# thelondonsmiths/Solex_ser_recon_EN

Hardware: AMD Instinct MI355X
Metric: SER frames/sec end-to-end (decode→clahe) + %HBM roofline, 1/2/4/8 MI355X (higher is better)
Workload: dtype u16

## Files before the change

### solex_ser_recon_en_amd/Solex_recon.py

```python
import contextlib
import functools
import math
import os
import queue
import sys
import threading

import numpy as np

from . import dist, ops, outputs, timing
from .device import DeviceImage, bind_thread, cpu_plan, default_device, to_device_u16
from .ellipse_to_circle import correct_image, ellipse_to_circle
from .fits_io import write_fits
from . import stages
from .solex_util import (as_uint16_image, clearlog, compute_mean_return_fit, correct_transversalium2_batch, extract_disks,
                         image_process_batch, logme, make_header, output_path, plots_enabled, removeVignette, savgol_taps,
                         savgol_window, write_complete, write_products)
from .video_reader import video_reader


WORKERS = 4


def _worker_count(workers, n_tasks):
# ... 498 lines not shown
                except BaseException as e:
                    with lock:
                        state['errors'].append((i, e))
                    break
            stream.synchronize()

    for k in range(n_workers):
        _Service.named('shg-scan-%s-%d' % (device, k)).jobs.put(functools.partial(run, k))
    for _ in range(n_workers):
        done.acquire()
    if state['errors']:
        raise min(state['errors'], key=lambda ie: ie[0])[1]


def _one_call_ok(rdr, options):
    if os.environ.get('SHG_SCAN_CALL', '1') == '0' or timing.enabled:
        return False
    if options.get('_shard_frames') or dist.is_sharded(rdr):
        return False
    if options['de-vignette'] or (options['transversalium'] and options.get('stubborn_transversalium')):
        return False
    return True


def scan_one_call(rdr, options):
    return _OneCall(rdr, options).run().finish()


class _OneCall:

    def __init__(self, rdr, options, pooled=False):
        self.rdr, self.options = rdr, options
        self.basefich0 = basefich0 = os.path.splitext(str(rdr.file))[0]
        options['basefich0'] = basefich0
        self.log = log = basefich0 + '_log.txt'
        clearlog(log, options)
        logme(log, options, 'Pixel shift : ' + str(options['shift']))
        options['shift_requested'] = options['shift']
        options['shift'] = list(dict.fromkeys([options['ellipse_fit_shift'], 0] + options['shift']))
        self.hdr = make_header(rdr)
        logme(log, options, 'Width, Height : ' + str(rdr.Width) + ' ' + str(rdr.Height))
        logme(log, options, 'Number of frames : ' + str(rdr.FrameCount))
        self.shifts = shifts = options['shift']
        self.requested = [sh in options['shift_requested'] for sh in shifts]
        self.plots = plots = plots_enabled(options)
        self.call = stages.ScanCall(rdr.device_stack(), shifts, self.requested, options, savgol_taps, want_plot_data=plots,
                                    want_fit_image=plots, own_buffers=pooled)

    def run(self):
        self.call.run()
        return self

    def submit(self, pool):
        self.call.submit(pool)
        return self

    def done(self):
        return self.call.done()

    def finish(self):
        from .ellipse_to_circle import _log_geometry, _warp_geometry
        rdr, options, hdr, log, basefich0 = self.rdr, self.options, self.hdr, self.log, self.basefich0
        shifts, requested, plots = self.shifts, self.requested, self.plots
        r, error = self.call.wait().collect()
        self.call = None
        _release_stack(rdr)
        phase = r['phase']
        if phase >= 1:
            mean_img = DeviceImage(r['mean'])
            y1, y2 = r['y1'], r['y2']
            if options['save_fit']:
                outputs.submit(write_fits, output_path(basefich0 + '_mean.fits', options), mean_img, hdr)
            logme(log, options, 'Vertical limits y1, y2 : ' + str(y1) + ' ' + str(y2))
            logme(log, options, lambda: 'Spectral line polynomial fit: ' + str(r['p']))
            if plots:
                rows = np.arange(y1, y2)
                good = r['mask_good']
                outputs.submit(outputs.plot_spectral_line, output_path(basefich0 + '_spectral_line_data.png', options), mean_img,
                               r['sharp'].astype(np.int64)[y1:y2][good], rows[good], r['fit'][:, 3], int(rdr.ih), (y2 - y1) // 20 + 1)
        disk_list = []
        if phase >= 2:
            hdr['NAXIS1'] = rdr.iw
            if options['save_fit'] or plots or (phase >= 3 and not r['limb_fitted'] and requested[0] and '_nolog' not in options):
                disk_list = [DeviceImage(r['disks'][i], minmax=r['extrema'][i]) for i in range(len(shifts))]
            if options.get('_keep_raw'):
                options['_raw_disks'] = [DeviceImage(r['disks'][i]) for i in range(len(shifts))]
            for i, disk in enumerate(disk_list):
                if options['save_fit'] and requested[i]:
                    outputs.submit(write_fits, output_path(basefich0 + '_shift=' + str(shifts[i]) + '_raw.fits', options), disk, hdr)
            if options['transversalium']:
                logme(log, options, 'Transversalium correction : ' + str(options['trans_strength']))
            else:
                logme(log, options, 'Transversalium disabled')
            logme(log, options, 'Mirror X : ' + str(options['flip_x']))
            logme(log, options, 'Post-rotation : ' + str(options['img_rotate']) + ' degrees')
            logme(log, options, f'Protus adjustment : {options["delta_radius"]}')
            logme(log, options, f'de-vignette : {options["de-vignette"]}')
        if phase >= 3:
            if r['limb_fitted']:
                options['ratio_fixe'] = r['ratio']
                _log_geometry(options, r['phi'], r['ratio'], r['theta_first'], np.array(r['circle'][:2]), r['circle'][2])
                print('sun borders found:' + str(r['borders']))
                options['slant_fix'] = math.degrees(r['phi'])
            elif requested[0] and '_nolog' not in options:
                ih_, n_ = disk_list[0].shape
                theta, inv_mat, _, _, _, origin, det = _warp_geometry(float(r['phi']), float(r['ratio']), int(ih_), int(n_))
                _log_geometry(options, r['phi'], r['ratio'], theta, (inv_mat @ np.array([-1.0, -1.0]).T).T - origin,
                              -1.0 * np.sqrt(np.abs(r['ratio'] / det)), known=False)
        if error is not None:
            raise error
        names = [basefich0 + '_shift=' + str(shifts[i]) for i in range(len(shifts)) if requested[i]]
        if plots and r['limb_fitted']:
            fix_img = r['frames'][0] if requested[0] else r['fit_image']
            outputs.submit(outputs.plot_ellipse_fit, output_path(basefich0 + '_shift=' + str(shifts[0]) + '_ellipse_fit.png', options),
                           disk_list[0], DeviceImage(fix_img), r['raw_X'], r['X_f'], r['outline'], r['borders'])
        if options['save_fit']:
            for j, basefich in enumerate(names):
                outputs.submit(write_fits, output_path(basefich + '_circular.fits', options), DeviceImage(r['frames'][j]), hdr)
        if options['transversalium']:
            for i, basefich in enumerate(names):
                c = r['factors'][i]
                options['_transversalium_cache'] = c
                if plots:
                    outputs.submit(outputs.plot_transversalium, output_path(basefich + '_transversalium_correction.png', options), c)
                if options['save_fit']:
                    outputs.submit(write_fits, output_path(basefich + '_detransversaliumed.fits', options), DeviceImage(r['detrans'][i]), hdr)
        if '_nolog' in options and not options['save_fit'] and options['img_rotate'] // 90 % 4 == 0:
            return [(DeviceImage(r['cc'][i]), DeviceImage(r['protus'][i])) for i in range(len(names))]
        results = [write_products(r['final'][i], r['cl1'][i], r['hc'][i], r['protus'][i], r['cc'][i], options, hdr, names[i])
                   for i in range(len(names))]
        for _ in names:
            write_complete(log, options)
        return results


def _writes_files(options):
    return not (options.get('_shard_frames') and dist.rank() != options.get('_owner', 0))


def solex_read(file, options):
    rdr = file if hasattr(file, 'device_stack') else video_reader(file)
    basefich0 = os.path.splitext(str(rdr.file))[0]
    options['basefich0'] = basefich0
    wopts = options if _writes_files(options) else dict(options, _nolog=True, save_fit=False)
    clearlog(basefich0 + '_log.txt', wopts)
    logme(basefich0 + '_log.txt', wopts, 'Pixel shift : ' + str(options['shift']))
    options['shift_requested'] = options['shift']
    options['shift'] = list(dict.fromkeys([options['ellipse_fit_shift'], 0] + options['shift']))
    if options.get('_shard_frames') and getattr(rdr, '_stack', None) is None:
        rdr.frame_range = dist.frame_block(int(rdr.FrameCount))
    hdr = make_header(rdr)
    ih, iw = rdr.ih, rdr.iw

    with timing.stage('mean_max+line_fit'):
        mean_img, fit, backup_y1, backup_y2 = compute_mean_return_fit(rdr, wopts, hdr, iw, ih, basefich0)
    with timing.stage('extract'):
        disks, extrema = extract_disks(rdr, fit, options['shift'], flip_x=bool(options['flip_x']), want_minmax=True,
                                       owner=options.get('_mosaic_to'))
    hdr['NAXIS1'] = iw

    disk_list = [DeviceImage(disks[i], minmax=None if extrema is None else extrema[i]) for i in range(disks.shape[0])]
    for i, disk in enumerate(disk_list):
        basefich = basefich0 + '_shift=' + str(options['shift'][i])
        flag_requested = options['shift'][i] in options['shift_requested']
        if wopts['save_fit'] and flag_requested:
            outputs.submit(write_fits, output_path(basefich + '_raw.fits', options), disk, hdr)
    return disk_list, (backup_y1, backup_y2), hdr
# ... 176 lines not shown
```

### solex_ser_recon_en_amd/csrc/extract.hip

```cpp
#include <stdlib.h>
#include <algorithm>
#include <type_traits>
#include "shg_common.h"

namespace shg {
thread_local bool t_minmax_slots_zeroed = false;
thread_local void* t_zero_with_fold = nullptr;
thread_local size_t t_zero_with_fold_words = 0;
thread_local void* t_prezeroed = nullptr;
}

namespace {

constexpr int TY = 64;
constexpr int TK = 64;
constexpr int TKP = TK + 2;
constexpr int SC_MAX = 4;

struct ExtractArgs {
    const void* stack;
    int n_frames;
    int64_t height, width, fstride;
    const int32_t* ind_l;
    const double *lw, *rw;
    int n_shifts;
    uint16_t* disks;
    int64_t row_pitch, plane_stride, n_cols, k_offset;
    int flip_x, vec_store;
    uint32_t* mm;
};

template <typename T, bool ROT, int BATCH, int SC> __global__ __launch_bounds__(256) void k_extract(const ExtractArgs kargs) {
    const T* __restrict__ stack = static_cast<const T*>(kargs.stack);
    const int n_frames = kargs.n_frames, n_shifts = kargs.n_shifts, flip_x = kargs.flip_x, vec_store = kargs.vec_store;
    const int64_t height = kargs.height, width = kargs.width, fstride = kargs.fstride, row_pitch = kargs.row_pitch, plane_stride = kargs.plane_stride,
                  n_cols = kargs.n_cols, k_offset = kargs.k_offset;
    const int32_t* __restrict__ ind_l = kargs.ind_l;
    const double* __restrict__ lw = kargs.lw;
    const double* __restrict__ rw = kargs.rw;
    uint16_t* __restrict__ disks = kargs.disks;
    uint32_t* __restrict__ mm = kargs.mm;
    __shared__ uint16_t tile[SC][TY][TKP];
    const int64_t ih = ROT ? width : height;
    const int lane = threadIdx.x & 63;
    const int wave = __builtin_amdgcn_readfirstlane(threadIdx.x >> 6);
    const int64_t c0 = (int64_t)blockIdx.x * TK;
    const int64_t y = (int64_t)blockIdx.y * TY + lane;
    const int s0 = blockIdx.z * SC;
    const int ns = min(SC, n_shifts - s0);
    const bool y_ok = y < ih;
    constexpr int scale = sizeof(T) == 1 ? 256 : 1;

    const int64_t yc = y_ok ? y : ih - 1;
    int il[SC];
    const double wl = lw[yc], wr = rw[yc];
    const double kl = wl * 0x1p+52, kr = wr * 0x1p+52;
    const bool fast = __all(fabs(wl) < 0x1p+900 && fabs(wr) < 0x1p+900) != 0;
#pragma unroll
    for (int s = 0; s < SC; ++s) il[s] = ind_l[(int64_t)(s0 + min(s, ns - 1)) * ih + yc];

    uint32_t off[SC], offr[SC];
    const int64_t step = ROT ? width : 1;
#pragma unroll
    for (int s = 0; s < SC; ++s) {
        off[s] = (uint32_t)((ROT ? (int64_t)il[s] * width + (width - 1 - yc) : yc * width + il[s]) * (int64_t)sizeof(T));
        offr[s] = off[s] + (uint32_t)(step * (int64_t)sizeof(T));
    }

    __shared__ uint32_t wred[4][SC][2];
    uint32_t vlo[SC], vhi[SC];
#pragma unroll
    for (int s = 0; s < SC; ++s) { vlo[s] = 0xffffu; vhi[s] = 0u; }

    for (int cb = wave; cb < TK; cb += 4 * BATCH) {
        T lv[BATCH][SC], rv[BATCH][SC];
        bool ok[BATCH];
#pragma unroll
        for (int i = 0; i < BATCH; ++i) {
            const int cc = cb + 4 * i;
            const int64_t col = c0 + cc;
            const int64_t k = (flip_x ? (n_cols - 1 - col) : col) - k_offset;
            ok[i] = cc < TK && col < n_cols && k >= 0 && k < n_frames;
            const char* f = reinterpret_cast<const char*>(stack + (ok[i] ? k : 0) * fstride);
#pragma unroll
            for (int s = 0; s < SC; ++s) {
                lv[i][s] = *reinterpret_cast<const T*>(f + off[s]);
                rv[i][s] = *reinterpret_cast<const T*>(f + offr[s]);
            }
        }
        auto blend = [&](auto fast_form) {
#pragma unroll
            for (int i = 0; i < BATCH; ++i) {
// ... 356 lines not shown
    constexpr int SEGS = TK / 8;
    const int seg = lane % SEGS;
    const int64_t col = c0 + seg * 8;
    const int64_t ka = (flip_x ? (n_cols - 1 - col) : col) - k_offset;
    const int64_t kb = (flip_x ? (n_cols - 1 - (col + 7)) : (col + 7)) - k_offset;
    const bool whole = a.vec_store && col + 8 <= n_cols && ka >= 0 && ka < n_frames && kb >= 0 && kb < n_frames;
    const int rows_here = (int)min((int64_t)TY, ih - (int64_t)by * TY);
    for (int d = wave; d < ns; d += NW) {
        const int plane = CONSEC ? a.plane_of[g0 + d] : g0 + d;
        uint16_t* dst0 = a.disks + (int64_t)plane * a.plane_stride + ((int64_t)by * TY) * a.row_pitch + col;
        uint32_t lo = 0xffffffffu, hi = 0u;
        if (whole) {
#pragma unroll 4
            for (int r = lane / SEGS; r < rows_here; r += 64 / SEGS) {
                const uint32_t* s32 = &btile[(d * TY + r) * DKW + seg * 4];
                const u32x4_t o = {s32[0], s32[1], s32[2], s32[3]};
                __builtin_nontemporal_store(o, reinterpret_cast<u32x4_t*>(dst0 + r * a.row_pitch));
                lo = pk_min_u16(pk_min_u16(lo, o.x), pk_min_u16(pk_min_u16(o.y, o.z), o.w));
                hi = pk_max_u16(pk_max_u16(hi, o.x), pk_max_u16(pk_max_u16(o.y, o.z), o.w));
            }
        } else {
            for (int r = lane / SEGS; r < rows_here; r += 64 / SEGS) {
                const uint16_t* src = reinterpret_cast<const uint16_t*>(&btile[(d * TY + r) * DKW + seg * 4]);
                uint16_t* dst = dst0 + r * a.row_pitch;
                for (int j = 0; j < 8; ++j) {
                    const int64_t cj = col + j;
                    const int64_t kj = (flip_x ? (n_cols - 1 - cj) : cj) - k_offset;
                    if (cj < n_cols && kj >= 0 && kj < n_frames) {
                        dst[j] = src[j];
                        lo = pk_min_u16(lo, src[j] * 0x10001u);
                        hi = pk_max_u16(hi, src[j] * 0x10001u);
                    }
                }
            }
        }
        if (a.mm) {
            lo = shg::wave_fold_u32(lo, [](uint32_t x, uint32_t y) { return pk_min_u16(x, y); });
            hi = shg::wave_fold_u32(hi, [](uint32_t x, uint32_t y) { return pk_max_u16(x, y); });
            const uint32_t l16 = min(lo & 0xffffu, lo >> 16), h16 = max(hi & 0xffffu, hi >> 16);
            if (lane == 0 && h16 >= l16) {
                const int slot = (int)((bx * 5u + by * 3u) & 63u);
                uint32_t* m = a.mm + ((int64_t)plane * 64 + slot) * 2;
                atomicMax(&m[0], 0xffffu - l16);
                atomicMax(&m[1], h16);
            }
        }
    }
}

template <bool CONSEC>
int launch_band(const BandArgs& ba, int bytes_per_px, int64_t ih, hipStream_t st) {
    const int S = ba.S;
    int G;
    if (CONSEC) {
        const int ng7 = (S + 6) / 7;
        G = std::max(4, (S + ng7 - 1) / ng7);
    } else {
        G = S <= 2 ? 2 : 4;
    }
    const int ng = (S + G - 1) / G;
    const dim3 grid(8u * (unsigned)ng, ((unsigned)ba.nx + 7u) / 8u, (unsigned)((ih + TY - 1) / TY));
    int status = SHG_E_UNSUPPORTED;
#define SHG_BAND(T, GV)                                                                                                                   \
    if (G == GV && bytes_per_px == (int)sizeof(T)) {                                                                                      \
        constexpr size_t lds = (size_t)GV * TY * (TK / 2 + 1) * 4;                                                                        \
        static const bool ok_ = lds <= 64 * 1024 || hipFuncSetAttribute(reinterpret_cast<const void*>(k_extract_band<T, GV, CONSEC>),    \
                                                                        hipFuncAttributeMaxDynamicSharedMemorySize, (int)lds) == hipSuccess; \
        if (!ok_) (void)hipGetLastError();                                                                                                \
        status = shg::launch_timed("extract", k_extract_band<T, GV, CONSEC>, grid, dim3(64 * BAND_NW), lds, st, nullptr, "k_extract_band", ba); \
    }
    if constexpr (CONSEC) {
        SHG_BAND(uint16_t, 4) SHG_BAND(uint16_t, 5) SHG_BAND(uint16_t, 6) SHG_BAND(uint16_t, 7)
        SHG_BAND(uint8_t, 4) SHG_BAND(uint8_t, 5) SHG_BAND(uint8_t, 6) SHG_BAND(uint8_t, 7)
    } else {
        SHG_BAND(uint16_t, 2) SHG_BAND(uint16_t, 4) SHG_BAND(uint8_t, 2) SHG_BAND(uint8_t, 4)
    }
#undef SHG_BAND
    return status;
}

struct FoldMinmaxArgs {
    const uint32_t* slots;
    uint32_t* out;
    int n_planes;
    uint32_t* zero;
    size_t zero_words;
};

__global__ __launch_bounds__(64) void k_fold_minmax(const FoldMinmaxArgs kargs) {
    const uint32_t* __restrict__ slots = kargs.slots;
    uint32_t* __restrict__ out = kargs.out;
    if ((int)blockIdx.x >= kargs.n_planes) {
        uint32_t* __restrict__ z = kargs.zero;
        const size_t stride = (size_t)(gridDim.x - kargs.n_planes) * 64;
        for (size_t i = (size_t)(blockIdx.x - kargs.n_planes) * 64 + threadIdx.x; i < kargs.zero_words; i += stride) z[i] = 0;
        return;
    }
    uint32_t a = slots[((int64_t)blockIdx.x * 64 + threadIdx.x) * 2], b = slots[((int64_t)blockIdx.x * 64 + threadIdx.x) * 2 + 1];
    a = shg::wave_fold_u32(a, [](uint32_t x, uint32_t y) { return x > y ? x : y; });
    b = shg::wave_fold_u32(b, [](uint32_t x, uint32_t y) { return x > y ? x : y; });
    if (threadIdx.x == 0) { out[blockIdx.x * 2] = 0xffffu - a; out[blockIdx.x * 2 + 1] = b; }
}

int launch_fold(uint32_t* minmax_slots, int n_shifts, hipStream_t st) {
    FoldMinmaxArgs fa{minmax_slots, minmax_slots + (int64_t)n_shifts * 64 * 2, n_shifts, nullptr, 0};
    unsigned extra = 0;
    if (shg::t_zero_with_fold && shg::t_zero_with_fold_words > 0) {
        fa.zero = static_cast<uint32_t*>(shg::t_zero_with_fold);
        fa.zero_words = shg::t_zero_with_fold_words;
        extra = (unsigned)std::min<size_t>((fa.zero_words + 1023) / 1024, 64);
    }
    const int e = shg::launch(k_fold_minmax, dim3((unsigned)n_shifts + extra), dim3(64), 0, st, fa, "k_fold_minmax");
    if (e == 0 && extra) shg::t_prezeroed = shg::t_zero_with_fold;
    shg::t_zero_with_fold = nullptr;
    shg::t_zero_with_fold_words = 0;
    return e;
}

}

extern "C" int shg_extract_columns(const void* stack, int64_t n_frames, int64_t height, int64_t width,
                                   int bytes_per_px, int64_t frame_stride_px, const int32_t* ind_l, const double* lw, const double* rw,
                                   int n_shifts, uint16_t* disks, int64_t row_pitch, int64_t plane_stride,
                                   int64_t n_cols, int64_t k_offset, int flip_x, shg_stream_t stream) {
    return shg_extract_columns_minmax(stack, n_frames, height, width, bytes_per_px, frame_stride_px, ind_l, lw, rw, n_shifts, disks,
                                      row_pitch, plane_stride, n_cols, k_offset, flip_x, nullptr, stream);
}

extern "C" int shg_extract_columns_minmax(const void* stack, int64_t n_frames, int64_t height, int64_t width,
                                          int bytes_per_px, int64_t frame_stride_px, const int32_t* ind_l, const double* lw, const double* rw,
                                          int n_shifts, uint16_t* disks, int64_t row_pitch, int64_t plane_stride,
                                          int64_t n_cols, int64_t k_offset, int flip_x, uint32_t* minmax_slots, shg_stream_t stream) {
    const bool slots_zeroed = shg::t_minmax_slots_zeroed;
    shg::t_minmax_slots_zeroed = false;
    SHG_REQUIRE(stack && ind_l && lw && rw && disks, SHG_E_ARG, "shg_extract_columns: null pointer");
    SHG_REQUIRE(n_frames > 0 && height > 0 && width > 0 && n_shifts > 0, SHG_E_ARG, "shg_extract_columns: empty input");
    SHG_REQUIRE(bytes_per_px == 1 || bytes_per_px == 2, SHG_E_ARG, "shg_extract_columns: bytes_per_px must be 1 or 2");
    SHG_REQUIRE(n_frames < (1ll << 31), SHG_E_UNSUPPORTED, "shg_extract_columns: too many frames");
    SHG_REQUIRE(n_cols >= n_frames && k_offset >= 0 && k_offset + n_frames <= n_cols, SHG_E_ARG,
                "shg_extract_columns: frames [%lld, %lld) do not fit %lld columns", (long long)k_offset,
                (long long)(k_offset + n_frames), (long long)n_cols);
    SHG_REQUIRE(row_pitch >= n_cols, SHG_E_ARG, "shg_extract_columns: row_pitch < n_cols");
    SHG_REQUIRE((height < width ? height : width) >= 2, SHG_E_ARG, "shg_extract_columns: spectral axis needs >= 2 pixels");
    SHG_REQUIRE(frame_stride_px == 0 || frame_stride_px >= height * width, SHG_E_ARG, "shg_extract_columns: frame stride smaller than a frame");
    SHG_REQUIRE(height * width * bytes_per_px < (1ll << 32), SHG_E_UNSUPPORTED, "shg_extract_columns: a frame of %lld x %lld samples is larger than 4 GiB",
                (long long)height, (long long)width);
    const int64_t fstride = frame_stride_px > 0 ? frame_stride_px : height * width;
    const bool rot = width > height;
    const int64_t ih = rot ? width : height;
    const int vec_store = ((reinterpret_cast<uintptr_t>(disks) & 15) == 0) && (row_pitch % 8 == 0) && (plane_stride % 8 == 0);
    static const int sc_env = [] { const char* e = getenv("SHG_EXT_SC"); return e ? atoi(e) : 0; }();
    const int sc = n_shifts <= 2 ? 2 : (sc_env == 2 ? 2 : SC_MAX);
    dim3 grid((unsigned)((n_cols + TK - 1) / TK), (unsigned)((ih + TY - 1) / TY), (unsigned)((n_shifts + sc - 1) / sc));
    hipStream_t st = shg::as_stream(stream);
    const int n = (int)n_frames;
    const ExtractArgs xa{stack, n, height, width, fstride, ind_l, lw, rw, n_shifts, disks, row_pitch, plane_stride, n_cols, k_offset, flip_x, vec_store, minmax_slots};
    int launch_status = 0;
#define EXT_LAUNCH_BS(T, ROT, B, SCV) launch_status = shg::launch_timed("extract", k_extract<T, ROT, B, SCV>, grid, dim3(256), 0, st, nullptr, "k_extract", xa)
#define EXT_LAUNCH_B(T, ROT, B) do { if (sc == 2) EXT_LAUNCH_BS(T, ROT, B, 2); else EXT_LAUNCH_BS(T, ROT, B, 4); } while (0)
#define EXT_LAUNCH(T, ROT)                                                 \
    switch (batch) {                                                       \
        case 1: EXT_LAUNCH_B(T, ROT, 1); break;                            \
        case 2: EXT_LAUNCH_B(T, ROT, 2); break;                            \
        case 8: EXT_LAUNCH_B(T, ROT, 8); break;                            \
        case 16: EXT_LAUNCH_B(T, ROT, 16); break;                          \
        default: EXT_LAUNCH_B(T, ROT, 4); break;                           \
    }
    static const int batch_env = [] { const char* e = getenv("SHG_EXT_BATCH"); return e ? atoi(e) : 0; }();
    const int batch2 = 4;
    const int batch = batch_env > 0 ? batch_env : (n_shifts > SC_MAX ? 8 : (n_shifts <= 2 ? batch2 : 4));
    if (minmax_slots && !slots_zeroed) {
        if (hipError_t e = hipMemsetAsync(minmax_slots, 0, (size_t)n_shifts * 64 * 2 * sizeof(uint32_t), st)) {
            shg::set_error("shg_extract_columns: memset: %s", hipGetErrorString(e));
            return (int)e;
        }
    }
    const bool general_only = [] { const char* e = getenv("SHG_EXT_GENERAL"); return e && atoi(e) != 0; }();
    if (rot && !general_only) {
        BandArgs ba{stack, n, height, width, fstride, ind_l, nullptr, lw, rw, n_shifts, disks, row_pitch, plane_stride, n_cols, k_offset, flip_x, vec_store,
                    minmax_slots, (int)((n_cols + TK - 1) / TK), {}};
        launch_status = launch_band<false>(ba, bytes_per_px, ih, st);
        if (launch_status) return launch_status;
        if (minmax_slots) return launch_fold(minmax_slots, n_shifts, st);
        return 0;
    }
    if (bytes_per_px == 2) {
        if (rot) EXT_LAUNCH(uint16_t, true) else EXT_LAUNCH(uint16_t, false)
    } else {
        if (rot) EXT_LAUNCH(uint8_t, true) else EXT_LAUNCH(uint8_t, false)
    }
#undef EXT_LAUNCH_B
#undef EXT_LAUNCH_BS
#undef EXT_LAUNCH
    if (launch_status) return launch_status;
    if (minmax_slots) return launch_fold(minmax_slots, n_shifts, st);
    return 0;
}

extern "C" int shg_extract_dense_fits(const int32_t* host_shifts, int n_shifts) {
    if (!host_shifts || n_shifts < 3 || n_shifts > DS_MAX) return 0;
    int lo = host_shifts[0], hi = host_shifts[0];
    for (int i = 1; i < n_shifts; ++i) { lo = host_shifts[i] < lo ? host_shifts[i] : lo; hi = host_shifts[i] > hi ? host_shifts[i] : hi; }
    if ((int64_t)hi - lo != n_shifts - 1) return 0;
    bool seen[DS_MAX] = {};
    for (int i = 0; i < n_shifts; ++i) {
        if (seen[host_shifts[i] - lo]) return 0;
        seen[host_shifts[i] - lo] = true;
    }
    return 1;
}

extern "C" int shg_extract_columns_dense(const void* stack, int64_t n_frames, int64_t height, int64_t width, int bytes_per_px,
                                         int64_t frame_stride_px, const int32_t* ind_l, const int32_t* base_col, const double* lw,
                                         const double* rw, const int32_t* host_shifts, int n_shifts, uint16_t* disks, int64_t row_pitch,
                                         int64_t plane_stride, int64_t n_cols, int64_t k_offset, int flip_x, uint32_t* minmax_slots,
                                         shg_stream_t stream) {
    const bool slots_zeroed = shg::t_minmax_slots_zeroed;
    shg::t_minmax_slots_zeroed = false;
    SHG_REQUIRE(stack && ind_l && base_col && lw && rw && host_shifts && disks, SHG_E_ARG, "shg_extract_columns_dense: null pointer");
    SHG_REQUIRE(n_frames > 0 && height > 0 && width > 0, SHG_E_ARG, "shg_extract_columns_dense: empty input");
    SHG_REQUIRE(shg_extract_dense_fits(host_shifts, n_shifts), SHG_E_UNSUPPORTED, "shg_extract_columns_dense: the shifts are not 3..%d consecutive integers", DS_MAX);
    SHG_REQUIRE(bytes_per_px == 1 || bytes_per_px == 2, SHG_E_ARG, "shg_extract_columns_dense: bytes_per_px must be 1 or 2");
    SHG_REQUIRE(n_frames < (1ll << 31), SHG_E_UNSUPPORTED, "shg_extract_columns_dense: too many frames");
    SHG_REQUIRE(n_cols >= n_frames && k_offset >= 0 && k_offset + n_frames <= n_cols, SHG_E_ARG, "shg_extract_columns_dense: frames do not fit the columns");
    SHG_REQUIRE(row_pitch >= n_cols, SHG_E_ARG, "shg_extract_columns_dense: row_pitch < n_cols");
    SHG_REQUIRE((height < width ? height : width) > n_shifts, SHG_E_UNSUPPORTED, "shg_extract_columns_dense: the spectral axis must be wider than the shift range");
    SHG_REQUIRE(frame_stride_px == 0 || frame_stride_px >= height * width, SHG_E_ARG, "shg_extract_columns_dense: frame stride smaller than a frame");
    const int64_t fstride = frame_stride_px > 0 ? frame_stride_px : height * width;
    const bool rot = width > height;
    const int64_t ih = rot ? width : height;
    const int vec_store = ((reinterpret_cast<uintptr_t>(disks) & 15) == 0) && (row_pitch % 8 == 0) && (plane_stride % 8 == 0);
    int lo = host_shifts[0];
    for (int i = 1; i < n_shifts; ++i) lo = host_shifts[i] < lo ? host_shifts[i] : lo;
    PlaneOfOffset po = {};
    for (int i = 0; i < n_shifts; ++i) po.v[host_shifts[i] - lo] = i;
    hipStream_t st = shg::as_stream(stream);
    if (minmax_slots && !slots_zeroed) {
        if (hipError_t e = hipMemsetAsync(minmax_slots, 0, (size_t)n_shifts * 64 * 2 * sizeof(uint32_t), st)) {
            shg::set_error("shg_extract_columns_dense: memset: %s", hipGetErrorString(e));
            return (int)e;
        }
    }
    const int n = (int)n_frames;
    if (rot) {
        BandArgs ba{stack, n, height, width, fstride, ind_l, base_col, lw, rw, n_shifts, disks, row_pitch, plane_stride, n_cols, k_offset, flip_x, vec_store,
                    minmax_slots, (int)((n_cols + TK - 1) / TK), {}};
        for (int i = 0; i < n_shifts; ++i) ba.plane_of[host_shifts[i] - lo] = (uint8_t)i;
        const int launch_status = launch_band<true>(ba, bytes_per_px, ih, st);
        if (launch_status) return launch_status;
        if (minmax_slots) return launch_fold(minmax_slots, n_shifts, st);
        return 0;
    }
    static const int shape = [] { const char* e = getenv("SHG_EXT_DENSE_SHAPE"); return e ? atoi(e) : 0; }();
#define SHG_DENSE(T, ROT, B, NW, DKV)                                                                                                               \
    do {                                                                                                                                            \
        static const bool ok_ = hipFuncSetAttribute(reinterpret_cast<const void*>(k_extract_dense<T, ROT, B, NW, DKV>),                            \
                                                    hipFuncAttributeMaxDynamicSharedMemorySize, 160 * 1024) == hipSuccess;                         \
        if (!ok_) (void)hipGetLastError();                                                                                                          \
        const size_t lds = (size_t)n_shifts * TY * (DKV + 2) * sizeof(uint16_t);                                                                    \
        dim3 grid((unsigned)((n_cols + DKV - 1) / DKV), (unsigned)((ih + TY - 1) / TY));                                                            \
        launch_status = shg::launch_timed("extract", k_extract_dense<T, ROT, B, NW, DKV>, grid, dim3(64 * NW), lds, st, nullptr, "k_extract_dense",      \
                                          static_cast<const T*>(stack), n, height, width, fstride, ind_l, base_col, lw, rw,                       \
                                          n_shifts, po, disks, row_pitch, plane_stride, n_cols, k_offset, flip_x, vec_store, minmax_slots);       \
    } while (0)
#define SHG_DENSE_S(T, ROT)                                                                  \
    do {                                                                                     \
        switch (shape) {                                                                     \
            case 1: SHG_DENSE(T, ROT, 4, 8, 32); break;                                      \
            case 2: SHG_DENSE(T, ROT, 2, 16, 32); break;                                     \
            case 3: SHG_DENSE(T, ROT, 4, 4, 16); break;                                      \
            case 4: SHG_DENSE(T, ROT, 2, 8, 16); break;                                      \
            case 5: SHG_DENSE(T, ROT, 2, 4, 8); break;                                       \
            case 6: SHG_DENSE(T, ROT, 4, 4, 32); break;                                      \
            default: SHG_DENSE(T, ROT, 4, 4, 16); break;                                     \
        }                                                                                    \
    } while (0)
    int launch_status = 0;
    if (bytes_per_px == 2) { if (rot) SHG_DENSE_S(uint16_t, true); else SHG_DENSE_S(uint16_t, false); }
    else { if (rot) SHG_DENSE_S(uint8_t, true); else SHG_DENSE_S(uint8_t, false); }
#undef SHG_DENSE_S
#undef SHG_DENSE
    if (launch_status) return launch_status;
    if (minmax_slots) return launch_fold(minmax_slots, n_shifts, st);
    return 0;
}
```

### solex_ser_recon_en_amd/csrc/limb_fused.hip

```cpp
#include <math.h>
#include <stdlib.h>
#include <algorithm>
#include "shg_common.h"

namespace {

#if defined(__HIP_DEVICE_COMPILE__) && !defined(__gfx950__)
#error "limb_fused.hip: published() relies on how gfx950 performs agent-scope atomics; use an acq_rel agent-scope fetch_add elsewhere"
#endif
__device__ __forceinline__ void published() {
    asm volatile("s_waitcnt vmcnt(0)" ::: "memory");
    __syncthreads();
}
__device__ __forceinline__ bool count_done(uint32_t* done, uint32_t total, int fence) {
    const uint32_t before = fence ? __hip_atomic_fetch_add(done, 1u, __ATOMIC_ACQ_REL, __HIP_MEMORY_SCOPE_AGENT)
                                  : __hip_atomic_fetch_add(done, 1u, __ATOMIC_RELAXED, __HIP_MEMORY_SCOPE_AGENT);
    return before == total - 1;
}
inline int limb_fence() {
    const char* v = getenv("SHG_LIMB_FENCE");
    return v && v[0] == '1';
}


// ... 9 lines not shown
    return (b >> 63) ? ~b : (b | 0x8000000000000000ull);
}
__device__ __forceinline__ double key_f64(uint64_t k) {
    const uint64_t b = (k >> 63) ? (k & 0x7fffffffffffffffull) : ~k;
    return __longlong_as_double((long long)b);
}

struct PrepLayout {
    int bits0, bits1;
    size_t hist0, hist1, coarse0, coarse1, acc, counts, done, zero_words;
    size_t keys5, keysk, total_words;
};

__host__ __device__ inline int bit_length(uint64_t v) {
    int b = 0;
    while (v) { ++b; v >>= 1; }
    return b;
}

PrepLayout prep_layout(int64_t sh, int64_t sw, int k) {
    PrepLayout L;
    const int kk = k > 5 ? k : 5;
    const int total_bits = bit_length((uint64_t)kk * kk * 16ull * 65535ull);
    L.bits1 = total_bits / 2;
    L.bits0 = total_bits - L.bits1;
    size_t off = 0;
    L.hist0 = off; off += (size_t)2 << L.bits0;
    L.hist1 = off; off += (size_t)4 << L.bits1;
    L.coarse0 = off; off += 2 * 256;
    L.coarse1 = off; off += 4 * 256;
    L.acc = off; off += 2 * (4 + 3 * FLOOD_SLOTS + 4 + FLOOD_SLOTS);
    L.counts = off; off += 20;
    L.done = off; off += 4;
    L.zero_words = off;
    off = (off + 63) / 64 * 64;
    const size_t n = (size_t)sh * (size_t)sw;
    L.keysk = off; off += (n + 63) / 64 * 64;
    L.keys5 = off; off += (n + 63) / 64 * 64;
    L.total_words = off;
    return L;
}

__device__ __forceinline__ void flush_hist(const uint32_t* lh, int bits, uint32_t* coarse_lds, uint32_t* __restrict__ fine,
                                           uint32_t* __restrict__ coarse, int tid, int nthreads) {
    for (int e = tid; e < 256; e += nthreads) coarse_lds[e] = 0;
    __syncthreads();
    const int shift = bits - 8;
    for (int e = tid; e < (1 << bits); e += nthreads) {
        const uint32_t c = lh[e];
        if (c) {
            atomicAdd(&fine[e], c);
            atomicAdd(&coarse_lds[e >> shift], c);
        }
    }
    __syncthreads();
    for (int e = tid; e < 256; e += nthreads)
        if (coarse_lds[e]) atomicAdd(&coarse[e], coarse_lds[e]);
}

__device__ __forceinline__ int refl101(int i, int n) {
    if (i < 0) i = -i;
    if (i >= n) i = 2 * n - 2 - i;
    return (i >= 0 && i < n) ? i : (int)shg::reflect101(i, n);
}

constexpr int BT = 16;
constexpr int NT1 = 1024;
struct ZeroWordsArgs {
    uint32_t* dst;
    size_t n_words;
};
__global__ __launch_bounds__(256) void k_zero_words(const ZeroWordsArgs kargs) {
    uint32_t* __restrict__ dst = kargs.dst;
    for (size_t i = (size_t)blockIdx.x * 256 + threadIdx.x; i < kargs.n_words; i += (size_t)gridDim.x * 256) dst[i] = 0;
}

struct LimbBlurArgs {
    const uint16_t* img;
    int h, w;
    int64_t pitch;
    int sh, sw, k, vec4;
    uint32_t *keysk, *keys5;
    unsigned long long* acc;
};
__global__ __launch_bounds__(256) void k_limb_blur(const LimbBlurArgs kargs) {
    const uint16_t* __restrict__ img = kargs.img;
    const int h = kargs.h, w = kargs.w, sh = kargs.sh, sw = kargs.sw, k = kargs.k, vec4 = kargs.vec4;
    const int64_t pitch = kargs.pitch;
    uint32_t* __restrict__ keysk = kargs.keysk;
    uint32_t* __restrict__ keys5 = kargs.keys5;
    unsigned long long* __restrict__ acc = kargs.acc;
    __shared__ uint32_t S[(BT + KMAX) * (BT + KMAX)];
    __shared__ uint32_t H[(BT + KMAX) * BT];
    __shared__ unsigned long long wsum[4];
    __shared__ uint32_t wmin[4];
    const int hl = max(k / 2, 2), hr = max(k - 1 - k / 2, 2);
    const int RH = BT + hl + hr, RW = RH;
    const int x0 = blockIdx.x * BT, y0 = blockIdx.y * BT;
    const int tid = threadIdx.x;
    uint32_t my_min = 0xffffffffu;
    unsigned long long own = 0;
    for (int e = tid; e < RH * RW; e += 256) {
        const int r = e / RW, c = e - r * RW;
        const int sy = refl101(y0 - hl + r, sh), sx = refl101(x0 - hl + c, sw);
        uint32_t s = 0;
        if (vec4 && sx * 4 + 4 <= w && sy * 4 + 4 <= h) {
            uint2 q[4];
#pragma unroll
            for (int j = 0; j < 4; ++j) q[j] = *reinterpret_cast<const uint2*>(img + (int64_t)(sy * 4 + j) * pitch + sx * 4);
#pragma unroll
            for (int j = 0; j < 4; ++j) s += (q[j].x & 0xffffu) + (q[j].x >> 16) + (q[j].y & 0xffffu) + (q[j].y >> 16);
        } else {
            for (int j = 0; j < 4; ++j) {
                const int y = sy * 4 + j;
                if (y >= h) break;
                for (int i = 0; i < 4; ++i) {
                    const int x = sx * 4 + i;
                    if (x < w) s += img[(int64_t)y * pitch + x];
                }
            }
        }
        S[e] = s;
        const int oy = y0 - hl + r, ox = x0 - hl + c;
        if (r >= hl && r < hl + BT && c >= hl && c < hl + BT && oy < sh && ox < sw) own += s;
    }
    own = shg::wave_sum((uint64_t)own);
    if ((tid & 63) == 0) wsum[tid >> 6] = own;
    const int n_arrays = k == 5 ? 1 : 2;
    for (int a = 0; a < n_arrays; ++a) {
        const int kw = a == 0 ? k : 5;
        uint32_t* keys = a == 0 ? keysk : keys5;
        __syncthreads();
        const int c_off = hl - kw / 2, r_lo = hl - kw / 2, r_n = BT + kw - 1;
        for (int e = tid; e < r_n * BT; e += 256) {
            const int r = r_lo + e / BT, x = e % BT;
            uint32_t s = 0;
            for (int j = 0; j < kw; ++j) s += S[r * RW + x + c_off + j];
            H[r * BT + x] = s;
        }
        __syncthreads();
        const int y = tid / BT, x = tid % BT;
        if (y0 + y < sh && x0 + x < sw) {
            uint32_t s = 0;
            for (int j = 0; j < kw; ++j) s += H[(r_lo + y + j) * BT + x];
            keys[(int64_t)(y0 + y) * sw + x0 + x] = s;
            if (a == 0) my_min = s;
        }
    }
    my_min = shg::wave_fold_u32(my_min, [](uint32_t x, uint32_t y) { return x < y ? x : y; });
    if ((tid & 63) == 0) wmin[tid >> 6] = my_min;
    __syncthreads();
    if (tid == 0) {
        const int slot = (blockIdx.y * gridDim.x + blockIdx.x) % FLOOD_SLOTS;
        const unsigned long long t = wsum[0] + wsum[1] + wsum[2] + wsum[3];
        if (t) atomicAdd(&acc[4 + 3 * slot], t);
        const uint32_t m = min(min(wmin[0], wmin[1]), min(wmin[2], wmin[3]));
        if (m != 0xffffffffu) atomicMax(&acc[4 + 3 * FLOOD_SLOTS + 4 + slot], ~f64_key(((double)m * kUnit) * (1.0 / ((double)k * (double)k))));
    }
}

__device__ __forceinline__ void wave_pick(const uint32_t* __restrict__ fine, const uint32_t* __restrict__ coarse, int bits, int64_t rank,
                                          int& digit, int64_t& below) {
    const int lane = threadIdx.x & 63;
    const int per = 1 << (bits - 8);
    int64_t c[4], local = 0;
#pragma unroll
    for (int j = 0; j < 4; ++j) {
        c[j] = __hip_atomic_load(&coarse[lane * 4 + j], __ATOMIC_RELAXED, __HIP_MEMORY_SCOPE_AGENT);
        local += c[j];
    }
    int64_t incl = shg::wave_scan((int64_t)local);
    int64_t excl = incl - local;
    int chunk = -1;
    int64_t base = 0;
    if (excl <= rank && rank < incl) {
#pragma unroll
        for (int j = 0; j < 4; ++j) {
            if (chunk < 0 && rank < excl + c[j]) { chunk = lane * 4 + j; base = excl; }
            excl += c[j];
        }
    }
    const unsigned long long owner = __ballot(chunk >= 0);
    const int src = owner ? __ffsll((long long)owner) - 1 : 0;
    chunk = __shfl(chunk, src);
    base = __shfl(base, src);
    const int64_t f = lane < per ? (int64_t)__hip_atomic_load(&fine[chunk * per + lane], __ATOMIC_RELAXED, __HIP_MEMORY_SCOPE_AGENT) : 0;
    int64_t fi = shg::wave_scan((int64_t)f);
    const int64_t fe = base + fi - f;
    const bool mine = lane < per && fe <= rank && rank < fe + f;
    const unsigned long long who = __ballot(mine);
    const int src2 = who ? __ffsll((long long)who) - 1 : 0;
    digit = chunk * per + src2;
    below = __shfl(fe, src2);
}

struct Ranks4 { int64_t rank[4]; int array[4]; double scale[4]; };

struct LimbSelect0Args {
    const uint32_t *keysk, *keys5;
    int64_t n;
    int bits0, bits1;
    uint32_t *hist0, *coarse0;
};
__global__ __launch_bounds__(256) void k_limb_select0(const LimbSelect0Args kargs) {
    const uint32_t* __restrict__ keysk = kargs.keysk;
    const uint32_t* __restrict__ keys5 = kargs.keys5;
    const int64_t n = kargs.n;
    const int bits0 = kargs.bits0, bits1 = kargs.bits1;
    uint32_t* __restrict__ hist0 = kargs.hist0;
    uint32_t* __restrict__ coarse0 = kargs.coarse0;
    extern __shared__ uint32_t lds[];
    __shared__ uint32_t lc[256];
    const int a = blockIdx.y;
    const uint32_t* __restrict__ v = a ? keys5 : keysk;
    for (int e = threadIdx.x; e < (1 << bits0); e += 256) lds[e] = 0;
    __syncthreads();
    const int64_t stride = (int64_t)gridDim.x * 256;
    for (int64_t base = (int64_t)blockIdx.x * 256 + threadIdx.x; base < n; base += 4 * stride) {
        uint32_t kk[4];
        bool ok[4];
#pragma unroll
        for (int u = 0; u < 4; ++u) { const int64_t i = base + u * stride; ok[u] = i < n; kk[u] = v[ok[u] ? i : 0]; }
#pragma unroll
        for (int u = 0; u < 4; ++u)
            if (ok[u]) atomicAdd(&lds[kk[u] >> bits1], 1u);
    }
    __syncthreads();
    flush_hist(lds, bits0, lc, hist0 + ((size_t)a << bits0), coarse0 + a * 256, threadIdx.x, 256);
}

struct LimbSelect1Args {
    const uint32_t *keysk, *keys5;
    int64_t n;
    Ranks4 p;
    int bits0, bits1;
    const uint32_t *hist0, *coarse0;
    uint32_t *hist1, *coarse1;
    double gamma;
    uint32_t* done;
    unsigned long long* acc;
    double* out4;
    int fence;
};
__global__ __launch_bounds__(256) void k_limb_select1(const LimbSelect1Args kargs) {
    const uint32_t* __restrict__ keysk = kargs.keysk;
    const uint32_t* __restrict__ keys5 = kargs.keys5;
    const int64_t n = kargs.n;
    const Ranks4& p = kargs.p;
    const int bits0 = kargs.bits0, bits1 = kargs.bits1;
    const uint32_t* __restrict__ hist0 = kargs.hist0;
    const uint32_t* __restrict__ coarse0 = kargs.coarse0;
    uint32_t* __restrict__ hist1 = kargs.hist1;
    uint32_t* __restrict__ coarse1 = kargs.coarse1;
    const double gamma = kargs.gamma;
    uint32_t* __restrict__ done = kargs.done;
    unsigned long long* __restrict__ acc = kargs.acc;
    double* __restrict__ out4 = kargs.out4;
    extern __shared__ uint32_t lds[];
    __shared__ uint32_t lc[256];
    __shared__ int last;
    __shared__ double val[4];
    const int pair = blockIdx.y;
    const uint32_t* __restrict__ v = p.array[pair] ? keys5 : keysk;
    int digit;
    int64_t below;
    wave_pick(hist0 + ((size_t)p.array[pair] << bits0), coarse0 + p.array[pair] * 256, bits0, p.rank[pair], digit, below);
    for (int e = threadIdx.x; e < (1 << bits1); e += 256) lds[e] = 0;
    __syncthreads();
    const uint32_t mask = (1u << bits1) - 1u;
    const int64_t stride = (int64_t)gridDim.x * 256;
    for (int64_t base = (int64_t)blockIdx.x * 256 + threadIdx.x; base < n; base += 4 * stride) {
        uint32_t kk[4];
        bool ok[4];
#pragma unroll
        for (int u = 0; u < 4; ++u) { const int64_t i = base + u * stride; ok[u] = i < n; kk[u] = v[ok[u] ? i : 0]; }
#pragma unroll
        for (int u = 0; u < 4; ++u)
            if (ok[u] && (int)(kk[u] >> bits1) == digit) atomicAdd(&lds[kk[u] & mask], 1u);
    }
    __syncthreads();
    flush_hist(lds, bits1, lc, hist1 + ((size_t)pair << bits1), coarse1 + pair * 256, threadIdx.x, 256);
    published();
    if (threadIdx.x == 0) last = count_done(done, gridDim.x * gridDim.y, kargs.fence);
    __syncthreads();
    if (!last) return;
    {
        const int q = threadIdx.x >> 6;
        int d0, d1;
        int64_t b0, b1;
        wave_pick(hist0 + ((size_t)p.array[q] << bits0), coarse0 + p.array[q] * 256, bits0, p.rank[q], d0, b0);
        wave_pick(hist1 + ((size_t)q << bits1), coarse1 + q * 256, bits1, p.rank[q] - b0, d1, b1);
        const uint64_t key = ((uint64_t)d0 << bits1) | (uint64_t)d1;
        if ((threadIdx.x & 63) == 0) val[q] = ((double)key * kUnit) * p.scale[q];
    }
    __syncthreads();
    __shared__ double vb_s;
    __shared__ int scan_s;
    __shared__ unsigned long long wmax[4];
    if (threadIdx.x == 0) {
        const double a = val[2], b = val[3], diff = b - a;
        const double very_bright = gamma >= 0.5 ? b - diff * (1.0 - gamma) : a + diff * gamma;
        out4[0] = val[0]; out4[1] = val[1]; out4[2] = a; out4[3] = b;
        acc[3] = (unsigned long long)__double_as_longlong(very_bright);
        vb_s = very_bright;
        scan_s = !(a < very_bright);
    }
    __syncthreads();
    const double very_bright = vb_s;
    unsigned long long hi = 0ull;
    if (scan_s) {
        const uint32_t* __restrict__ vk = p.array[2] ? keys5 : keysk;
        for (int64_t i = threadIdx.x; i < n; i += 256) {
// ... 351 lines not shown
    if (threadIdx.x == 0) base = part[0] + part[1] + part[2] + part[3];
    __syncthreads();
    for (int xb = 0; xb < w; xb += 256) {
        const int x = xb + threadIdx.x;
        int root = -1, hi = 0;
        if (x < w) {
            const int i = y * w + x;
            const int l = L[i];
            if (l >= 0) {
                root = g_find(L, l);
                hi = (mask[i] >> 1) & 1;
            }
        }
        const unsigned long long m = __ballot(root >= 0);
        if (lane == 0) wave_cnt[wave] = __popcll(m);
        __syncthreads();
        int off = base;
        for (int i = 0; i < wave; ++i) off += wave_cnt[i];
        if (root >= 0) {
            const int pos = off + __popcll(m & ((1ull << lane) - 1ull));
            comp[1 + pos] = y * w + x;
            comp[1 + n + pos] = root | (hi << 30);
        }
        __syncthreads();
        if (threadIdx.x == 0) base += wave_cnt[0] + wave_cnt[1] + wave_cnt[2] + wave_cnt[3];
        __syncthreads();
    }
    if (y == h - 1 && threadIdx.x == 0) comp[0] = base;
}

size_t canny_tile_lds(int R) {
    const int FW = TW + 4 + 2 * R, FH = TH + 4 + 2 * R, VW = FW, VH = TH + 4, SW = TW + 4, MW = TW + 2, MH = TH + 2;
    return (size_t)(((VH + 7) & ~7) + VH * VW + VH * SW + 3 * MH * MW) * 8 + (size_t)TH * TW * 4 + (size_t)FH * FW;
}

}

extern "C" int shg_limb_fused_fits(int64_t sh, int64_t sw, int k) {
    return sh > 2 && sw > 2 && sh * sw < (1ll << 30) && k >= 1 && k <= KMAX;
}

size_t shg::limb_prepare_zero_words(int64_t h, int64_t w) {
    const int64_t sh = (h + 3) / 4, sw = (w + 3) / 4;
    const int k = (int)((double)sh * 0.01);
    if (!shg_limb_fused_fits(sh, sw, k)) return 0;
    return prep_layout(sh, sw, k).zero_words;
}

extern "C" size_t shg_limb_prepare_workspace_bytes(int64_t sh, int64_t sw, int k) {
    if (!shg_limb_fused_fits(sh, sw, k)) return 0;
    return prep_layout(sh, sw, k).total_words * 4;
}

extern "C" int shg_limb_prepare(const uint16_t* img, int64_t h, int64_t w, int64_t pitch, int k, const int64_t* host_ranks4, double gamma99,
                                double* packed, const uint32_t** keys_out, void* workspace, size_t workspace_bytes, shg_stream_t stream) {
    SHG_REQUIRE(img && host_ranks4 && packed && keys_out && workspace, SHG_E_ARG, "shg_limb_prepare: null pointer");
    SHG_REQUIRE(h > 0 && w > 0 && pitch >= w, SHG_E_ARG, "shg_limb_prepare: bad image size");
    const int64_t sh = (h + 3) / 4, sw = (w + 3) / 4, n = sh * sw;
    SHG_REQUIRE(shg_limb_fused_fits(sh, sw, k), SHG_E_UNSUPPORTED, "shg_limb_prepare: a %d x %d window on %lld x %lld is outside the fused path", k, k,
                (long long)sh, (long long)sw);
    SHG_REQUIRE(gamma99 >= 0.0 && gamma99 <= 1.0, SHG_E_ARG, "shg_limb_prepare: gamma %g outside [0, 1]", gamma99);
    const PrepLayout lay = prep_layout(sh, sw, k);
    SHG_REQUIRE(workspace_bytes >= lay.total_words * 4, SHG_E_WORKSPACE, "shg_limb_prepare: workspace too small");
    SHG_REQUIRE((reinterpret_cast<uintptr_t>(workspace) & 7) == 0, SHG_E_ARG, "shg_limb_prepare: workspace not 8-byte aligned");
    for (int i = 0; i < 4; ++i) SHG_REQUIRE(host_ranks4[i] >= 0 && host_ranks4[i] < n, SHG_E_ARG, "shg_limb_prepare: rank outside the image");
    hipStream_t st = shg::as_stream(stream);
    uint32_t* ws = static_cast<uint32_t*>(workspace);
    uint32_t *hist0 = ws + lay.hist0, *hist1 = ws + lay.hist1, *coarse0 = ws + lay.coarse0, *coarse1 = ws + lay.coarse1;
    uint32_t *counts = ws + lay.counts, *done = ws + lay.done;
    unsigned long long* acc = reinterpret_cast<unsigned long long*>(ws + lay.acc);
    uint32_t *keysk = ws + lay.keysk, *keys5 = k == 5 ? keysk : ws + lay.keys5;
    double* out4 = reinterpret_cast<double*>(acc + 4 + 3 * FLOOD_SLOTS);
    SHG_PROF("limb_prepare", st);
    if (shg::t_prezeroed == workspace) {
        shg::t_prezeroed = nullptr;
    } else if (int e = shg::launch(k_zero_words, dim3((unsigned)std::min<size_t>((lay.zero_words + 255) / 256, 64)), dim3(256), 0, st, ZeroWordsArgs{ws, lay.zero_words}, "k_zero_words")) {
        return e;
    }
    Ranks4 p;
    const double scale_k = 1.0 / ((double)k * (double)k), scale_5 = 1.0 / 25.0;
    for (int i = 0; i < 4; ++i) { p.rank[i] = host_ranks4[i]; p.array[i] = (i < 2 && k != 5) ? 1 : 0; p.scale[i] = (i < 2) ? scale_5 : scale_k; }
    dim3 grid1((unsigned)((sw + BT - 1) / BT), (unsigned)((sh + BT - 1) / BT));
    const int vec4 = (reinterpret_cast<uintptr_t>(img) & 7) == 0 && pitch % 4 == 0;
    if (int e = shg::launch(k_limb_blur, grid1, dim3(256), 0, st, LimbBlurArgs{img, (int)h, (int)w, pitch, (int)sh, (int)sw, k, vec4, keysk, keys5, acc}, "k_limb_blur")) return e;
    static const bool lds_ok = [] {
        return hipFuncSetAttribute(reinterpret_cast<const void*>(k_limb_select0), hipFuncAttributeMaxDynamicSharedMemorySize, 128 * 1024) == hipSuccess &&
               hipFuncSetAttribute(reinterpret_cast<const void*>(k_limb_select1), hipFuncAttributeMaxDynamicSharedMemorySize, 128 * 1024) == hipSuccess;
    }();
    if (!lds_ok) (void)hipGetLastError();
    int64_t blocks = (n + 2047) / 2048;
    if (blocks > 256) blocks = 256;
    if (int e = shg::launch(k_limb_select0, dim3((unsigned)blocks, k == 5 ? 1u : 2u), dim3(256), ((size_t)1 << lay.bits0) * 4, st,
                           LimbSelect0Args{keysk, keys5, n, lay.bits0, lay.bits1, hist0, coarse0}, "k_limb_select0"))
        return e;
    if (int e = shg::launch(k_limb_select1, dim3((unsigned)blocks, 4u), dim3(256), ((size_t)1 << lay.bits1) * 4, st,
                           LimbSelect1Args{keysk, keys5, n, p, lay.bits0, lay.bits1, hist0, coarse0, hist1, coarse1, gamma99, done, acc, out4, limb_fence()}, "k_limb_select1"))
        return e;
    *keys_out = keysk;
    return shg::launch(k_limb_flood_hist, dim3((unsigned)blocks), dim3(256), 0, st, LimbFloodHistArgs{keysk, n, scale_k, acc, out4, counts, done + 1, packed, limb_fence()}, "k_limb_flood_hist");
}

extern "C" size_t shg_limb_edges_workspace_bytes(int64_t sh, int64_t sw) {
    if (sh <= 0 || sw <= 0) return 0;
    const size_t n = (size_t)sh * (size_t)sw, tiles_x = (size_t)((sw + TW - 1) / TW);
    return ((n + 255) / 256 * 256) + n * 4 + (size_t)sh * tiles_x * 4 + 256;
}

extern "C" int shg_limb_edges(const uint32_t* keys, int64_t sh, int64_t sw, int k, double flood_thresh, const double* host_gauss_weights,
                              int radius, double low, double high, int32_t* comp, void* workspace, size_t workspace_bytes, shg_stream_t stream) {
    SHG_REQUIRE(keys && host_gauss_weights && comp && workspace, SHG_E_ARG, "shg_limb_edges: null pointer");
    SHG_REQUIRE(sh > 2 && sw > 2 && sh * sw < (1ll << 30) && k >= 1, SHG_E_ARG, "shg_limb_edges: bad image size");
    SHG_REQUIRE(radius >= 0 && radius <= MAXR, SHG_E_UNSUPPORTED, "shg_limb_edges: Gaussian radius %d > %d", radius, MAXR);
    SHG_REQUIRE(workspace_bytes >= shg_limb_edges_workspace_bytes(sh, sw), SHG_E_WORKSPACE, "shg_limb_edges: workspace too small");
    GaussW g;
    g.radius = radius;
    for (int i = 0; i < 2 * radius + 1; ++i) g.w[i] = host_gauss_weights[i];
    const size_t n = (size_t)sh * (size_t)sw;
    const int tiles_x = (int)((sw + TW - 1) / TW);
    uint8_t* mask = static_cast<uint8_t*>(workspace);
    int* L = reinterpret_cast<int*>(mask + (n + 255) / 256 * 256);
    int* row_counts = L + n;
    hipStream_t st = shg::as_stream(stream);
    SHG_PROF("limb_edges", st);
    dim3 grid((unsigned)tiles_x, (unsigned)((sh + TH - 1) / TH));
    static const bool lds_ok = hipFuncSetAttribute(reinterpret_cast<const void*>(k_limb_canny_tile), hipFuncAttributeMaxDynamicSharedMemorySize, 160 * 1024) == hipSuccess;
    if (!lds_ok) (void)hipGetLastError();
    if (int e = shg::launch(k_limb_canny_tile, grid, dim3(NT1), canny_tile_lds(radius), st,
                           LimbCannyArgs{keys, (int)sh, (int)sw, 1.0 / ((double)k * (double)k), flood_thresh, g, low, high, mask, L, row_counts, tiles_x}, "k_limb_canny_tile"))
        return e;
    {
        const int64_t tops = ((sh + TH - 1) / TH) * sw, sides = 2 * (int64_t)tiles_x * sh;
        if (int e = shg::launch(k_limb_border_merge, dim3((unsigned)((std::max(tops, sides) + 255) / 256), 2u), dim3(256), 0, st, LimbBorderArgs{mask, (int)sh, (int)sw, L}, "k_limb_border_merge"))
            return e;
    }
    return shg::launch(k_limb_emit, dim3((unsigned)sh), dim3(256), 0, st, LimbEmitArgs{mask, L, (int)sh, (int)sw, row_counts, tiles_x, (int)n, comp}, "k_limb_emit");
}
```

### solex_ser_recon_en_amd/csrc/scan.hip

```cpp
#include <math.h>
#include <string.h>
#include <atomic>
#include <vector>
#include "shg_common.h"

namespace {

constexpr size_t kAlign = 256;
inline size_t up(size_t b) { return (b + kAlign - 1) / kAlign * kAlign; }
inline int64_t round64(int64_t v) { return (v + 63) / 64 * 64; }
inline int64_t floor_div(int64_t a, int64_t b) { int64_t q = a / b; return (a % b != 0 && ((a < 0) != (b < 0))) ? q - 1 : q; }

const double kRadToDeg = 180.0 / 3.141592653589793238462643383279502884;
const double kDegToRad = 3.141592653589793238462643383279502884 / 180.0;

std::atomic<shg_savgol_taps_fn> g_taps_fn{nullptr};

#define SCAN_TRY(expr)                  \
    do {                                \
        if (int e_ = (expr)) return e_; \
    } while (0)

struct Regions {
    size_t mean_ws, extract_ws, limb_ws, mean_pin, extract_pin, limb_pin, process_pin;
// ... 90 lines not shown
        SHG_REQUIRE(fabs(c[0]) < 9e15 && fabs(c[1]) < 9e15 && fabs(c[2]) < 9e15, SHG_E_VALUE, "cannot convert float NaN / infinity to integer (disk circle)");
        const int64_t r = (int64_t)c[2] + rq->delta_radius;
        if (r > 0) { pl->disc[0] = (int64_t)c[0]; pl->disc[1] = (int64_t)c[1]; pl->disc[2] = r; }
    }
    memcpy(rs->disc3, pl->disc, sizeof(rs->disc3));
    return 0;
}

}

extern "C" int shg_host_set_savgol_taps(shg_savgol_taps_fn fn) {
    g_taps_fn.store(fn);
    return 0;
}

extern "C" size_t shg_scan_workspace_bytes(const shg_scan_request* rq) {
    if (!rq || rq->height <= 0 || rq->width <= 0 || rq->n_frames <= 0 || rq->n_shifts <= 0 || !rq->host_requested) return 0;
    const Regions r = regions(rq);
    return r.mean_ws + r.extract_ws + r.limb_ws + kAlign;
}

extern "C" size_t shg_scan_host_bytes(const shg_scan_request* rq) {
    if (!rq || rq->height <= 0 || rq->width <= 0 || rq->n_frames <= 0 || rq->n_shifts <= 0 || !rq->host_requested) return 0;
    const Regions r = regions(rq);
    return r.mean_pin + r.extract_pin + r.limb_pin + r.process_pin + kAlign;
}

extern "C" int shg_scan_prelaunch(const shg_scan_request* rq, shg_stream_t after, int* launched) {
    SHG_REQUIRE(rq && launched, SHG_E_ARG, "shg_scan_prelaunch: null pointer");
    *launched = 0;
    if (rq->struct_bytes != sizeof(shg_scan_request) || rq->start_phase != 0 || !rq->stack || !rq->workspace || rq->n_frames <= 0 ||
        rq->height <= 0 || rq->width <= 0 || rq->n_shifts <= 0 || (rq->bytes_per_px != 1 && rq->bytes_per_px != 2))
        return 0;
    const Regions rg = regions(rq);
    const size_t acc = shg_accumulate_workspace_bytes(rq->n_frames, rq->height, rq->width, rq->bytes_per_px);
    if (rq->workspace_bytes < rg.mean_ws || acc == 0 || acc > rg.mean_ws) return 0;
    return shg_pass_a_prelaunch(rq->stack, rq->n_frames, rq->height, rq->width, rq->bytes_per_px, rq->frame_stride_px, rq->workspace, acc, after,
                                launched);
}

extern "C" int shg_scan_file(const shg_scan_request* rq, shg_scan_result* rs, shg_stream_t stream) {
    SHG_HOST_TIME("scan_file");
    SHG_REQUIRE(rq && rs, SHG_E_ARG, "shg_scan_file: null pointer");
    SHG_REQUIRE(rq->struct_bytes == sizeof(shg_scan_request), SHG_E_ARG, "shg_scan_file: the caller's shg_scan_request has %u bytes, the library's %zu",
                rq->struct_bytes, sizeof(shg_scan_request));
    SHG_REQUIRE(rq->stack && rq->host_shifts && rq->host_requested && rq->mean_out && rq->max_out && rq->disks && rq->minmax_slots &&
                rq->workspace && rq->host_pinned && rq->host_fit, SHG_E_ARG, "shg_scan_file: null pointer in the request");
    SHG_REQUIRE(rq->n_frames > 0 && rq->height > 0 && rq->width > 0 && rq->n_shifts > 0, SHG_E_ARG, "shg_scan_file: empty input");
    SHG_REQUIRE(rq->disk_pitch >= rq->n_frames && rq->disk_plane_stride > 0, SHG_E_ARG, "shg_scan_file: bad disk layout");
    SHG_REQUIRE(rq->start_phase == 0 || rq->start_phase == 3, SHG_E_ARG, "shg_scan_file: start_phase must be 0 or 3");
    const int64_t ih = slit_rows(rq), n_cols = rq->n_frames;
    const int S = rq->n_shifts;
    const int64_t k = n_requested(rq);
    const bool limb = fits_limb(rq);
    SHG_REQUIRE(!limb || (rq->host_gauss_taps && rq->host_points && rq->host_flags && rq->points_cap > 0), SHG_E_ARG,
                "shg_scan_file: the limb fit needs host_gauss_taps, host_points, host_flags");
    const Regions rg = regions(rq);
    char* ws = static_cast<char*>(rq->workspace);
    char* pin = static_cast<char*>(rq->host_pinned);
    const size_t ws_fixed = rg.mean_ws + rg.extract_ws + rg.limb_ws;
    SHG_REQUIRE(rq->workspace_bytes >= ws_fixed, SHG_E_WORKSPACE, "shg_scan_file: workspace %zu < %zu bytes", rq->workspace_bytes, ws_fixed);
    SHG_REQUIRE(rq->host_pinned_bytes >= rg.mean_pin + rg.extract_pin + rg.limb_pin + rg.process_pin, SHG_E_WORKSPACE,
                "shg_scan_file: pinned staging area %zu < %zu bytes", rq->host_pinned_bytes, rg.mean_pin + rg.extract_pin + rg.limb_pin + rg.process_pin);
    char* mean_ws = ws;
    char* extract_ws = mean_ws + rg.mean_ws;
    char* limb_ws = extract_ws + rg.extract_ws;
    char* process_ws = limb_ws + rg.limb_ws;
    char* mean_pin = pin;
    char* extract_pin = mean_pin + rg.mean_pin;
    char* limb_pin = extract_pin + rg.extract_pin;
    char* process_pin = limb_pin + rg.limb_pin;

    if (rq->start_phase == 0) {
        memset(rs, 0, sizeof(*rs));
        rs->fit_image_off = rs->frames_off = rs->detrans_off = rs->products_off = rs->results_off = -1;
        int64_t y12[2];
        SCAN_TRY(shg_stage_mean_fit(rq->stack, rq->n_frames, rq->height, rq->width, rq->bytes_per_px, rq->frame_stride_px, nullptr, nullptr,
                                    rq->n_frames, rq->mean_out, rq->max_out, y12, rs->p4, rq->host_fit, rq->host_trace_sharp, rq->host_mask_good,
                                    mean_ws, rg.mean_ws, mean_pin, rg.mean_pin, stream));
        rs->y1 = y12[0];
        rs->y2 = y12[1];
        rs->phase_done = 1;
        if (limb) {
            shg::t_zero_with_fold = limb_ws;
            shg::t_zero_with_fold_words = shg::limb_prepare_zero_words(ih, n_cols);
        }
        const int extract_status = shg_stage_extract(rq->stack, rq->n_frames, rq->height, rq->width, rq->bytes_per_px, rq->frame_stride_px, rq->host_fit,
                                                     rq->host_shifts, S, rq->disks, rq->disk_pitch, rq->disk_plane_stride, n_cols, 0, rq->flip_x,
                                                     rq->minmax_slots, extract_ws, rg.extract_ws, extract_pin, rg.extract_pin, stream);
        shg::t_zero_with_fold = nullptr;
        shg::t_zero_with_fold_words = 0;
        if (extract_status) { shg::t_prezeroed = nullptr; return extract_status; }
        rs->phase_done = 2;
        bool later_disks = false;
        for (int i = 1; i < S; ++i) later_disks = later_disks || rq->host_requested[i];
        double mat3[9], inv[4], origin[2], det;
        if (limb) {
            int64_t dims[2];
            const int limb_status = shg_stage_limb_fit(rq->disks, ih, n_cols, rq->disk_pitch, rq->host_gauss_taps, rq->host_points, rq->host_flags, rq->points_cap,
                                                       rs->counts3, rs->geom16, dims, rq->host_outline200, limb_ws, rg.limb_ws, limb_pin, rg.limb_pin, stream);
            shg::t_prezeroed = nullptr;
            if (limb_status) return limb_status;
            const double* g = rs->geom16;
            rs->limb_fitted = 1;
            rs->phi = g[3];
            rs->ratio = g[4];
            memcpy(rs->circle3, g + 5, 3 * sizeof(double));
            memcpy(rs->borders4, g + 8, 4 * sizeof(double));
            memcpy(rs->h_first, g + 12, 3 * sizeof(double));
            rs->theta_first = g[15];
            rs->out_h = dims[0];
            rs->out_w = dims[1];
            memcpy(rs->h_rest, rs->h_first, sizeof(rs->h_rest));
            rs->theta_rest = rs->theta_first;
            if (later_disks) {
                const double phi_again = (rs->phi * kRadToDeg) * kDegToRad;
                int64_t oh, ow;
                SCAN_TRY(shg_host_warp_geometry(phi_again, rs->ratio, ih, n_cols, mat3, inv, origin, &det, &rs->theta_rest, &oh, &ow));
                SHG_REQUIRE(oh == rs->out_h && ow == rs->out_w, SHG_E_VALUE, "process_frames: the frames must share one shape and row pitch");
                memcpy(rs->h_rest, mat3, 3 * sizeof(double));
            }
        } else {
            rs->ratio = isnan(rq->ratio_fixe) ? 1.0 : rq->ratio_fixe;
            rs->phi = isnan(rq->slant_fix_deg) ? 0.0 : rq->slant_fix_deg * kDegToRad;
            SCAN_TRY(shg_host_warp_geometry(rs->phi, rs->ratio, ih, n_cols, mat3, inv, origin, &det, &rs->theta_first, &rs->out_h, &rs->out_w));
            memcpy(rs->h_first, mat3, 3 * sizeof(double));
            memcpy(rs->h_rest, mat3, 3 * sizeof(double));
            rs->theta_rest = rs->theta_first;
            rs->circle3[0] = rs->circle3[1] = rs->circle3[2] = -1;
            shg::t_prezeroed = nullptr;
        }
        rs->phase_done = 3;
    } else {
        SHG_REQUIRE(rs->phase_done == 3, SHG_E_ARG, "shg_scan_file: nothing to resume (phase_done = %d)", rs->phase_done);
    }

    Plan pl;
    SCAN_TRY(make_plan(rq, rs, &pl));
    const int64_t out_h = rs->out_h, out_w = rs->out_w;
    SHG_REQUIRE(out_h > 0 && out_w > 0, SHG_E_VALUE, "correct_image: empty output (%lld x %lld)", (long long)out_h, (long long)out_w);
    const int64_t frame_pitch = round64(out_w);
    const int64_t prod_w = pl.crop_w > 0 ? pl.crop_w : out_w, prod_pitch = round64(prod_w);
    const bool fit_image = rq->want_fit_image && !rq->host_requested[0];
    const bool detrans = rq->transversalium && rq->keep_detrans && k > 0;
    const size_t frame_bytes = up((size_t)out_h * frame_pitch * 2), prod_bytes = up((size_t)out_h * prod_pitch * 2);
    size_t off = 0;
    rs->fit_image_off = fit_image ? (int64_t)off : -1;
    off += fit_image ? frame_bytes : 0;
    rs->frames_off = k > 0 ? (int64_t)off : -1;
    off += (size_t)k * frame_bytes;
    rs->detrans_off = detrans ? (int64_t)off : -1;
    off += detrans ? (size_t)k * frame_bytes : 0;
    rs->products_off = k > 0 ? (int64_t)off : -1;
    off += (size_t)k * 3 * prod_bytes;
    rs->results_off = k > 0 ? 0 : -1;
    rs->needed_results_bytes = (size_t)k * 2 * prod_bytes;
    rs->frame_pitch = frame_pitch;
    rs->n_out = k;
    rs->prod_w = prod_w;
    rs->prod_pitch = prod_pitch;
    rs->needed_arena_bytes = off;
    const size_t process_ws_bytes = k > 0 ? up(shg_stage_process_workspace_bytes(k, out_h, out_w, pl.crop_w, rq->tiles)) : 0;
    rs->needed_workspace_bytes = ws_fixed + process_ws_bytes;
    if (rq->arena_bytes < rs->needed_arena_bytes || (off > 0 && !rq->arena) || rq->results_bytes < rs->needed_results_bytes ||
        (k > 0 && !rq->results) || rq->workspace_bytes < rs->needed_workspace_bytes) {
        shg::set_error("shg_scan_file: the corrected images are %lld x %lld: arena %zu of %zu bytes, results %zu of %zu bytes, workspace %zu of "
                       "%zu bytes -- grow them and call again with start_phase = 3", (long long)out_h, (long long)out_w, rq->arena_bytes,
                       rs->needed_arena_bytes, rq->results_bytes, rs->needed_results_bytes, rq->workspace_bytes, rs->needed_workspace_bytes);
        return SHG_E_WORKSPACE;
    }
    SHG_REQUIRE(((reinterpret_cast<uintptr_t>(rq->arena) | reinterpret_cast<uintptr_t>(rq->results)) & 255) == 0, SHG_E_ARG,
                "shg_scan_file: arenas not 256-byte aligned");
    char* arena = static_cast<char*>(rq->arena);
    char* results = static_cast<char*>(rq->results);
    const uint32_t* extrema = rq->minmax_slots + (size_t)S * 128;
    std::vector<const uint16_t*> w_src;
    std::vector<uint16_t*> w_dst;
    std::vector<const uint32_t*> w_mm;
    std::vector<double> w_h;
    auto add_warp = [&](int i, uint16_t* dst) {
        const double* hr = i == 0 ? rs->h_first : rs->h_rest;
        w_src.push_back(rq->disks + (size_t)i * rq->disk_plane_stride);
        w_dst.push_back(dst);
        w_mm.push_back(extrema + 2 * i);
        w_h.insert(w_h.end(), hr, hr + 3);
    };
    if (fit_image) add_warp(0, reinterpret_cast<uint16_t*>(arena + rs->fit_image_off));
    std::vector<const uint16_t*> frames((size_t)k);
    std::vector<uint16_t*> det((size_t)k), prod[5];
    for (auto& v : prod) v.resize((size_t)k);
    int64_t j = 0;
    for (int i = 0; i < S; ++i) {
        if (!rq->host_requested[i]) continue;
        uint16_t* f = reinterpret_cast<uint16_t*>(arena + rs->frames_off + (size_t)j * frame_bytes);
        add_warp(i, f);
        frames[j] = f;
        if (detrans) det[j] = reinterpret_cast<uint16_t*>(arena + rs->detrans_off + (size_t)j * frame_bytes);
        for (int p = 0; p < 3; ++p) prod[p][j] = reinterpret_cast<uint16_t*>(arena + rs->products_off + ((size_t)j * 3 + p) * prod_bytes);
        for (int p = 0; p < 2; ++p) prod[3 + p][j] = reinterpret_cast<uint16_t*>(results + ((size_t)j * 2 + p) * prod_bytes);
        ++j;
    }
    if (!w_src.empty())
        SCAN_TRY(shg::warp_rows_batch(w_src.data(), (int64_t)w_src.size(), ih, n_cols, rq->disk_pitch, w_h.data(), w_dst.data(), out_h, out_w, frame_pitch,
                                      w_mm.data(), stream));
    if (k > 0) {
        SCAN_TRY(shg_stage_process_frames(frames.data(), k, out_h, out_w, frame_pitch, rq->transversalium, pl.trans_circle, pl.trans_borders,
                                          pl.taps_ptr, pl.window, rq->host_factors, pl.crop_w, pl.sx0, pl.dx0, pl.ncopy, rq->clip_limit, rq->tiles,
                                          pl.disc[0], pl.disc[1], pl.disc[2], detrans ? det.data() : nullptr, frame_pitch, prod[0].data(),
                                          prod[1].data(), prod[2].data(), prod[3].data(), prod[4].data(), prod_pitch, process_ws, process_ws_bytes,
                                          process_pin, rg.process_pin, stream));
    }
    rs->phase_done = 4;
    return 0;
}
```

### solex_ser_recon_en_amd/csrc/shg_common.h

```cpp
#pragma once
#include <hip/hip_runtime.h>
#include <hip/hip_ext.h>
#include <stdint.h>
#include <stdio.h>
#include <type_traits>
#include "../../include/shg_hip.h"

namespace shg {

void set_error(const char* fmt, ...);

inline int check_launch(const char* what) {
    hipError_t e = hipGetLastError();
    if (e != hipSuccess) {
        set_error("%s: %s", what, hipGetErrorString(e));
        return (int)e;
    }
    return 0;
}


template <typename A>
struct same_type { using type = A; };
template <typename A>
inline int launch(void (*k)(A), dim3 grid, dim3 block, size_t lds, hipStream_t st, const typename same_type<A>::type& a, const char* what) {
    hipLaunchKernelGGL(k, grid, block, lds, st, a);
    return check_launch(what);
}

struct TimedEvents { hipEvent_t start = nullptr, stop = nullptr; bool sampled = false; };
int timed_begin(const char* tag, bool want_done, TimedEvents* ev);
void timed_end(const char* tag, hipStream_t st, const TimedEvents& ev, bool launched, hipEvent_t* done);
void event_release(hipEvent_t e);
template <typename... P>
inline int launch_timed(const char* tag, void (*k)(P...), dim3 grid, dim3 block, size_t lds, hipStream_t st, hipEvent_t* done, const char* what,
                        typename same_type<P>::type... a) {
    TimedEvents ev;
    if (int e = timed_begin(tag, done != nullptr, &ev)) return e;
    int r;
    if (ev.start || ev.stop) {
        void* args[] = {static_cast<void*>(&a)...};
        const hipError_t le = hipExtLaunchKernel(reinterpret_cast<const void*>(k), grid, block, args, lds, st, ev.start, ev.stop, 0);
        r = check_launch(what);
        if (r == 0 && le != hipSuccess) { set_error("%s: %s", what, hipGetErrorString(le)); r = (int)le; }
    } else {
        hipLaunchKernelGGL(k, grid, block, lds, st, a...);
        r = check_launch(what);
    }
    timed_end(tag, st, ev, r == 0, done);
    return r;
}

#define SHG_REQUIRE(cond, code, ...)            \
    do {                                        \
        if (!(cond)) {                          \
            shg::set_error(__VA_ARGS__);        \
            return (code);                      \
        }                                       \
    } while (0)

inline hipStream_t as_stream(shg_stream_t s) { return reinterpret_cast<hipStream_t>(s); }

typedef int (*lane_launch_fn)(hipStream_t st, void* arg, hipEvent_t* done);
int on_frame_pass_lane(hipStream_t st, lane_launch_fn launch, void* arg);

extern thread_local bool t_minmax_slots_zeroed;
extern thread_local void* t_zero_with_fold;
extern thread_local size_t t_zero_with_fold_words;
extern thread_local void* t_prezeroed;
size_t limb_prepare_zero_words(int64_t h, int64_t w);
int prelaunch_on_lane(hipStream_t after, lane_launch_fn launch, void* arg, hipEvent_t* done);

struct ProfScope {
    ProfScope(const char* tag, hipStream_t st);
    ~ProfScope();
    int slot;
    hipStream_t stream;
    unsigned generation;
};
#define SHG_PROF(tag, st) shg::ProfScope shg_prof_scope_(tag, st)

struct HostScope {
    explicit HostScope(const char* tag);
    ~HostScope();
    const char* tag;
    double t0;
};
#define SHG_HOST_CAT2(a, b) a##b
#define SHG_HOST_CAT(a, b) SHG_HOST_CAT2(a, b)
#define SHG_HOST_TIME(tag) shg::HostScope SHG_HOST_CAT(shg_host_scope_, __LINE__)(tag)

constexpr int kMaxBatch = 32;
template <int N>
struct PtrBatchN {
    const void* p[N];
    template <typename T>
    __device__ __forceinline__ T* at(int i) const { return static_cast<T*>(const_cast<void*>(p[i])); }
};
using PtrBatch = PtrBatchN<kMaxBatch>;
template <int N, typename T>
inline PtrBatchN<N> make_batch_n(T* const* host_ptrs, int first, int count) {
    PtrBatchN<N> b = {};
    for (int i = 0; i < count && i < N; ++i) b.p[i] = host_ptrs[first + i];
    return b;
}
template <typename T>
inline PtrBatch make_batch(T* const* host_ptrs, int first, int count) { return make_batch_n<kMaxBatch>(host_ptrs, first, count); }

int rowpair_stats_batch(const uint16_t* const* host_imgs, int64_t k, int64_t h, int64_t w, int64_t pitch, int64_t y1, int64_t y2,
                        const int32_t* xa, const int32_t* xb, const double* row_factor, double* out, double* out_mirror, shg_stream_t stream);
int scale_rows_batch(const uint16_t* const* host_imgs, int64_t k, int64_t h, int64_t w, int64_t pitch, const double* c,
                     const double* row_factor, uint16_t* const* host_dsts, int64_t dst_pitch, shg_stream_t stream);
int crop_pad_batch(const uint16_t* const* host_srcs, int64_t k, int64_t h, int64_t w, int64_t pitch, uint16_t* const* host_dsts, int64_t nw,
                   int64_t dst_pitch, int64_t sx0, int64_t dx0, int64_t n, int32_t fill, shg_stream_t stream);
int contrast_products_batch(const uint16_t* const* host_frames, int64_t frame_pitch, const uint16_t* const* host_cl1, int64_t cl1_pitch,
                            int64_t k, int64_t h, int64_t w, const double* host_lo_hi6, uint16_t* const* host_hc, uint16_t* const* host_protus,
                            uint16_t* const* host_cc, int64_t dst_pitch, int64_t disc_x0, int64_t disc_y0, int64_t disc_r, shg_stream_t stream,
                            const double* stats5 = nullptr, double g_bright = 0.0, double g_dark = 0.0, double* mirror5 = nullptr);
int warp_rows_batch(const uint16_t* const* host_srcs, int64_t k, int64_t h, int64_t w, int64_t src_pitch, const double* host_h3,
                    uint16_t* const* host_dsts, int64_t out_h, int64_t out_w, int64_t dst_pitch, const uint32_t* const* host_minmax2,
                    shg_stream_t stream);
struct FrameSource {
    const uint16_t* const* host_raw;
    int64_t raw_pitch;
    const double* factors;
    int64_t sx0, dx0, ncopy;
};
bool contrast_stats_batches(int64_t h, int64_t w, int tiles, double clip_limit);
int contrast_stats_batch(const uint16_t* const* host_frames, int64_t k, int64_t h, int64_t w, int64_t pitch, double clip_limit, int tiles,
                         uint16_t* const* host_cl1, int64_t cl1_pitch, const int64_t* ranks_frame2, const int64_t* ranks_cl13, double* out5,
                         void* workspace, size_t workspace_bytes, shg_stream_t stream, const FrameSource* from = nullptr);

constexpr int kWave = 64;
constexpr int kCUs = 256;

__device__ __forceinline__ int lane_id() { return threadIdx.x & (kWave - 1); }

template <typename Op>
__device__ __forceinline__ uint32_t wave_fold_u32(uint32_t v, Op op) {
    v = op(v, (uint32_t)__builtin_amdgcn_update_dpp((int)v, (int)v, 0xB1, 0xf, 0xf, false));
    v = op(v, (uint32_t)__builtin_amdgcn_update_dpp((int)v, (int)v, 0x4E, 0xf, 0xf, false));
    v = op(v, (uint32_t)__builtin_amdgcn_update_dpp((int)v, (int)v, 0x141, 0xf, 0xf, false));
    v = op(v, (uint32_t)__builtin_amdgcn_update_dpp((int)v, (int)v, 0x140, 0xf, 0xf, false));
    const uint32_t r0 = (uint32_t)__builtin_amdgcn_readlane((int)v, 0), r1 = (uint32_t)__builtin_amdgcn_readlane((int)v, 16),
                   r2 = (uint32_t)__builtin_amdgcn_readlane((int)v, 32), r3 = (uint32_t)__builtin_amdgcn_readlane((int)v, 48);
    return op(op(r0, r1), op(r2, r3));
}

template <typename Op>
__device__ __forceinline__ uint64_t wave_fold_u64(uint64_t v, Op op) {
    auto step = [&](auto ctrl) {
        const int lo = __builtin_amdgcn_update_dpp((int)(uint32_t)v, (int)(uint32_t)v, decltype(ctrl)::value, 0xf, 0xf, false);
        const int hi = __builtin_amdgcn_update_dpp((int)(v >> 32), (int)(v >> 32), decltype(ctrl)::value, 0xf, 0xf, false);
        v = op(v, ((uint64_t)(uint32_t)hi << 32) | (uint32_t)lo);
    };
    step(std::integral_constant<int, 0xB1>{});
    step(std::integral_constant<int, 0x4E>{});
    step(std::integral_constant<int, 0x141>{});
    step(std::integral_constant<int, 0x140>{});
    auto at = [&](int l) {
        return ((uint64_t)(uint32_t)__builtin_amdgcn_readlane((int)(v >> 32), l) << 32) | (uint32_t)__builtin_amdgcn_readlane((int)(uint32_t)v, l);
    };
    return op(op(at(0), at(16)), op(at(32), at(48)));
}
__device__ __forceinline__ uint64_t wave_sum(uint64_t v) { return wave_fold_u64(v, [](uint64_t a, uint64_t b) { return a + b; }); }
__device__ __forceinline__ uint64_t wave_min(uint64_t v) { return wave_fold_u64(v, [](uint64_t a, uint64_t b) { return a < b ? a : b; }); }
__device__ __forceinline__ uint64_t wave_max(uint64_t v) { return wave_fold_u64(v, [](uint64_t a, uint64_t b) { return a > b ? a : b; }); }

template <int CTRL>
__device__ __forceinline__ int dpp_get(int v, int fallback) {
    return __builtin_amdgcn_update_dpp(fallback, v, CTRL, 0xf, 0xf, false);
}
__device__ __forceinline__ int wave_sum(int v) {
    v += dpp_get<0xB1>(v, v);
    v += dpp_get<0x4E>(v, v);
    v += dpp_get<0x141>(v, v);
    v += dpp_get<0x140>(v, v);
    return (__builtin_amdgcn_readlane(v, 0) + __builtin_amdgcn_readlane(v, 16)) + (__builtin_amdgcn_readlane(v, 32) + __builtin_amdgcn_readlane(v, 48));
}
__device__ __forceinline__ uint32_t wave_sum(uint32_t v) { return (uint32_t)wave_sum((int)v); }
__device__ __forceinline__ int sum_of_8_lanes(int v) {
    v += dpp_get<0xB1>(v, v);
    v += dpp_get<0x4E>(v, v);
    v += dpp_get<0x141>(v, v);
    return v;
}
__device__ __forceinline__ uint32_t sum_of_32_lanes(uint32_t u) {
    int v = (int)u;
    v += dpp_get<0xB1>(v, v);
    v += dpp_get<0x4E>(v, v);
    v += dpp_get<0x141>(v, v);
    v += dpp_get<0x140>(v, v);
    const int lo = __builtin_amdgcn_readlane(v, 0) + __builtin_amdgcn_readlane(v, 16), hi = __builtin_amdgcn_readlane(v, 32) + __builtin_amdgcn_readlane(v, 48);
    return (uint32_t)((threadIdx.x & 32) ? hi : lo);
}
__device__ __forceinline__ int wave_scan(int v) {
    v += dpp_get<0x111>(v, 0);
    v += dpp_get<0x112>(v, 0);
    v += dpp_get<0x114>(v, 0);
    v += dpp_get<0x118>(v, 0);
    const int t0 = __builtin_amdgcn_readlane(v, 15), t1 = __builtin_amdgcn_readlane(v, 31), t2 = __builtin_amdgcn_readlane(v, 47);
    const int lane = threadIdx.x & 63;
    return v + (lane >= 16 ? t0 : 0) + (lane >= 32 ? t1 : 0) + (lane >= 48 ? t2 : 0);
}
// ... 27 lines not shown
```

### solex_ser_recon_en_amd/csrc/stages.hip

```cpp
#include <math.h>
#include <stdlib.h>
#include <string.h>
#include <algorithm>
#include <vector>
#include "shg_common.h"

namespace {

constexpr size_t kAlign = 256;
inline size_t up(size_t b) { return (b + kAlign - 1) / kAlign * kAlign; }

struct Arena {
    char* base;
    size_t cap, off;
    Arena(void* p, size_t bytes) : base(static_cast<char*>(p)), cap(bytes), off(0) {}
    template <typename T>
    T* take(size_t count) {
        const size_t b = up(count * sizeof(T));
        if (!base || off + b > cap) return nullptr;
        T* p = reinterpret_cast<T*>(base + off);
        off += b;
        return p;
    }
};

#define STAGE_TRY(expr)            \
    do {                           \
        if (int e_ = (expr)) return e_; \
    } while (0)

#define STAGE_SYNC(st, who)                                                \
    do {                                                                   \
        SHG_HOST_TIME("sync");                                             \
        if (hipError_t se_ = hipStreamSynchronize(st)) {                   \
            shg::set_error("%s: %s", who, hipGetErrorString(se_));         \
            return (int)se_;                                               \
        }                                                                  \
    } while (0)

struct WordsArgs {
    uint32_t* dst;
    const uint32_t* src;
    size_t n_words;
    uint32_t* zero;
    size_t zero_words;
};
__global__ __launch_bounds__(256) void k_words(const WordsArgs kargs) {
    uint32_t* __restrict__ dst = kargs.dst;
    const uint32_t* __restrict__ src = kargs.src;
    const size_t n_words = kargs.n_words;
    for (size_t i = (size_t)blockIdx.x * 256 + threadIdx.x; i < n_words; i += (size_t)gridDim.x * 256) dst[i] = src[i];
}

__global__ __launch_bounds__(256) void k_words_zero(const WordsArgs kargs) {
    uint32_t* __restrict__ dst = kargs.dst;
    const uint32_t* __restrict__ src = kargs.src;
    const size_t n_words = kargs.n_words, zero_words = kargs.zero_words;
    uint32_t* __restrict__ zero = kargs.zero;
    for (size_t i = (size_t)blockIdx.x * 256 + threadIdx.x; i < n_words; i += (size_t)gridDim.x * 256) dst[i] = src[i];
    for (size_t i = (size_t)blockIdx.x * 256 + threadIdx.x; i < zero_words; i += (size_t)gridDim.x * 256) zero[i] = 0;
}

__global__ __launch_bounds__(256) void k_edge_list(const int32_t* __restrict__ comp, int64_t n, int32_t* __restrict__ dst) {
    const int64_t m = comp[0];
    for (int64_t i = (int64_t)blockIdx.x * 256 + threadIdx.x; i < m; i += (int64_t)gridDim.x * 256) {
        dst[1 + i] = comp[1 + i];
        dst[1 + n + i] = comp[1 + n + i];
    }
    if (blockIdx.x == 0 && threadIdx.x == 0) dst[0] = (int32_t)m;
}

inline int move_words(void* dst, const void* src, size_t bytes, hipStream_t st) {
    const size_t n_words = (bytes + 3) / 4;
    if (n_words == 0) return 0;
    const unsigned blocks = (unsigned)std::min<size_t>((n_words + 255) / 256, 64);
    return shg::launch(k_words, dim3(blocks), dim3(256), 0, st, WordsArgs{static_cast<uint32_t*>(dst), static_cast<const uint32_t*>(src), n_words, nullptr, 0}, "k_words");
}

struct Staging {
    char* host;
    char* dev;
    template <typename T>
    T* on_device(T* host_ptr) const { return reinterpret_cast<T*>(dev + (reinterpret_cast<char*>(host_ptr) - host)); }
};

inline int map_staging(void* host_pinned, Staging* out, const char* who) {
    void* d = nullptr;
    hipError_t e = hipHostGetDevicePointer(&d, host_pinned, 0);
    if (e != hipSuccess || !d) {
        (void)hipGetLastError();
        shg::set_error("%s: host_pinned is not page-locked, GPU-mapped memory (hipHostMalloc / hipHostRegister): %s", who,
                       e != hipSuccess ? hipGetErrorString(e) : "no device address");
        return SHG_E_ARG;
    }
    out->host = static_cast<char*>(host_pinned);
    out->dev = static_cast<char*>(d);
    return 0;
}

inline int64_t slit_rows(int64_t height, int64_t width) { return width > height ? width : height; }
inline int64_t spectral_cols(int64_t height, int64_t width) { return width > height ? height : width; }

}

extern "C" size_t shg_stage_mean_fit_workspace_bytes(int64_t n_frames, int64_t height, int64_t width, int bytes_per_px) {
    if (height <= 0 || width <= 0) return 0;
    const size_t hw = (size_t)height * (size_t)width, ih = (size_t)slit_rows(height, width);
    const size_t acc = n_frames > 0 ? shg_accumulate_workspace_bytes(n_frames, height, width, bytes_per_px) : 0;
    return up(acc) + up(hw * 8) + up(hw * 2) + up(hw * 2) + up(hw * 4) + up(ih * 8) + up(2 * ih * 4) + kAlign;
}

extern "C" size_t shg_stage_mean_fit_host_bytes(int64_t height, int64_t width) {
    if (height <= 0 || width <= 0) return 0;
    const size_t ih = (size_t)slit_rows(height, width);
    return up(ih * 8) + up(2 * ih * 4);
}

extern "C" int shg_stage_mean_fit(const void* stack, int64_t n_frames, int64_t height, int64_t width, int bytes_per_px,
                                  int64_t frame_stride_px, const uint64_t* sum_in, const uint16_t* max_in, int64_t n_total,
                                  uint16_t* mean_out, uint16_t* max_out, int64_t* host_y12, double* host_p4, double* host_fit,
                                  int32_t* host_trace_sharp, uint8_t* host_mask_good, void* workspace, size_t workspace_bytes,
                                  void* host_pinned, size_t host_pinned_bytes, shg_stream_t stream) {
    SHG_HOST_TIME("stage mean_fit");
    SHG_REQUIRE(mean_out && max_out && host_y12 && host_p4 && host_fit && workspace && host_pinned, SHG_E_ARG,
                "shg_stage_mean_fit: null pointer");
    SHG_REQUIRE((sum_in == nullptr) == (max_in == nullptr), SHG_E_ARG, "shg_stage_mean_fit: sum_in and max_in go together");
    SHG_REQUIRE(sum_in || stack, SHG_E_ARG, "shg_stage_mean_fit: neither a stack nor its sums");
    SHG_REQUIRE(height > 0 && width > 0 && n_total > 0, SHG_E_ARG, "shg_stage_mean_fit: empty input");
    const int64_t ih = slit_rows(height, width), iw = spectral_cols(height, width);
    const size_t hw = (size_t)height * (size_t)width;
    hipStream_t st = shg::as_stream(stream);
    Arena dev(workspace, workspace_bytes), pin(host_pinned, host_pinned_bytes);
    const size_t acc_bytes = sum_in ? 0 : shg_accumulate_workspace_bytes(n_frames, height, width, bytes_per_px);
    char* acc_ws = dev.take<char>(acc_bytes ? acc_bytes : 1);
    uint64_t* sum = dev.take<uint64_t>(hw);
    uint16_t* mx = dev.take<uint16_t>(hw);
    uint16_t* blur = dev.take<uint16_t>(hw);
    uint32_t* tmp = dev.take<uint32_t>(hw);
    double* row_means = dev.take<double>((size_t)ih);
    int32_t* traces = dev.take<int32_t>(2 * (size_t)ih);
    double* h_means = pin.take<double>((size_t)ih);
    int32_t* h_traces = pin.take<int32_t>(2 * (size_t)ih);
    SHG_REQUIRE(acc_ws && sum && mx && blur && tmp && row_means && traces, SHG_E_WORKSPACE, "shg_stage_mean_fit: workspace too small");
    SHG_REQUIRE(h_means && h_traces, SHG_E_WORKSPACE, "shg_stage_mean_fit: pinned staging area too small");
    Staging stg;
    STAGE_TRY(map_staging(host_pinned, &stg, "shg_stage_mean_fit"));
    row_means = stg.on_device(h_means);
    traces = stg.on_device(h_traces);

    if (!sum_in) {
        SHG_REQUIRE(n_total == n_frames, SHG_E_ARG, "shg_stage_mean_fit: n_total %lld != %lld frames of the stack", (long long)n_total, (long long)n_frames);
        STAGE_TRY(shg_accumulate_mean_max(stack, n_frames, height, width, bytes_per_px, frame_stride_px, mean_out, max_out, acc_ws, acc_bytes, stream));
    } else {
        STAGE_TRY(shg_finalize_mean_max(sum_in, max_in, n_total, height, width, bytes_per_px, mean_out, max_out, stream));
    }
    if (shg_blur_fits_fused(iw, 5)) {
        STAGE_TRY(shg_blur_row_mean_u16(max_out, ih, iw, 5, 5, row_means, stream));
    } else {
        STAGE_TRY(shg_box_blur_u16(max_out, ih, iw, 5, 5, blur, tmp, stream));
        STAGE_TRY(shg_row_mean_u16(blur, ih, iw, row_means, stream));
    }
    STAGE_SYNC(st, "shg_stage_mean_fit");
    int64_t y1, y2;
    STAGE_TRY(shg_host_detect_bord(h_means, ih, &y1, &y2));
    const int64_t clip = (int64_t)((double)(y2 - y1) * 0.05);
    y1 = std::min(ih - 1, y1 + clip);
    y2 = std::max<int64_t>(0, y2 - clip);
    host_y12[0] = y1;
    host_y12[1] = y2;
    const int blur_w = 25, blur_h = (int)((double)(y2 - y1) * 0.01);
    const int64_t lo = blur_w / 2, hi = iw + (-(blur_w + 1) / 2);
    if (blur_h > 0 && shg_blur_fits_fused(iw, blur_h)) {
        STAGE_TRY(shg_blur_argmin_u16(mean_out, ih, iw, blur_w, blur_h, lo, hi, traces, traces + ih, stream));
    } else {
        STAGE_TRY(shg_box_blur_u16(mean_out, ih, iw, blur_w, blur_h, blur, tmp, stream));
        STAGE_TRY(shg_row_argmin_u16(blur, ih, iw, lo, hi, traces, stream));
        STAGE_TRY(shg_row_argmin_u16(mean_out, ih, iw, 0, iw, traces + ih, stream));
    }
    STAGE_SYNC(st, "shg_stage_mean_fit");
    if (host_trace_sharp) memcpy(host_trace_sharp, h_traces + ih, (size_t)ih * 4);
    return shg_host_line_fit(h_traces, h_traces + ih, ih, y1, y2, (int32_t)lo, host_p4, host_fit, host_mask_good);
}

extern "C" size_t shg_stage_extract_workspace_bytes(int64_t height, int64_t width, int n_shifts) {
    if (height <= 0 || width <= 0 || n_shifts <= 0) return 0;
    const size_t ih = (size_t)slit_rows(height, width);
    return up((size_t)n_shifts * ih * 4) + up(2 * ih * 8) + up(ih * 4);
}

extern "C" int shg_stage_extract(const void* stack, int64_t n_frames, int64_t height, int64_t width, int bytes_per_px,
                                 int64_t frame_stride_px, const double* host_fit, const int32_t* host_shifts, int n_shifts,
                                 uint16_t* disks, int64_t row_pitch, int64_t plane_stride, int64_t n_cols, int64_t k_offset,
                                 int flip_x, uint32_t* minmax_slots, void* workspace, size_t workspace_bytes, void* host_pinned,
                                 size_t host_pinned_bytes, shg_stream_t stream) {
    SHG_HOST_TIME("stage extract");
    SHG_REQUIRE(stack && host_fit && host_shifts && disks && workspace && host_pinned, SHG_E_ARG, "shg_stage_extract: null pointer");
    SHG_REQUIRE(height > 0 && width > 0 && n_shifts > 0, SHG_E_ARG, "shg_stage_extract: empty input");
    const int64_t ih = slit_rows(height, width), iw = spectral_cols(height, width);
    Arena dev(workspace, workspace_bytes), pin(host_pinned, host_pinned_bytes);
    int32_t* ind_l = dev.take<int32_t>((size_t)n_shifts * ih);
    double* w2 = dev.take<double>(2 * (size_t)ih);
    int32_t* base = dev.take<int32_t>((size_t)ih);
    int32_t* h_ind = pin.take<int32_t>((size_t)n_shifts * ih);
    double* h_w2 = pin.take<double>(2 * (size_t)ih);
    int32_t* h_base = pin.take<int32_t>((size_t)ih);
    SHG_REQUIRE(ind_l && w2 && base, SHG_E_WORKSPACE, "shg_stage_extract: workspace too small");
    SHG_REQUIRE(h_ind && h_w2 && h_base, SHG_E_WORKSPACE, "shg_stage_extract: pinned staging area too small");
    STAGE_TRY(shg_host_column_plan(host_fit, ih, iw, host_shifts, n_shifts, h_ind, h_w2, h_w2 + ih));
    const int dense_mode = [] { const char* v = getenv("SHG_EXT_DENSE"); return v ? atoi(v) : 1; }();
    const bool dense = dense_mode > 0 && iw > n_shifts && shg_extract_dense_fits(host_shifts, n_shifts);
    if (dense) {
        int lo = host_shifts[0];
        for (int i = 1; i < n_shifts; ++i) lo = std::min(lo, (int)host_shifts[i]);
        for (int64_t y = 0; y < ih; ++y) {
            const double v = host_fit[y * 4] + 1.0 * (double)lo;
            h_base[y] = (v == v && v > -1e9 && v < 1e9) ? (int32_t)(int64_t)v : INT32_MIN;
        }
    }
    hipStream_t st = shg::as_stream(stream);
    Staging stg;
    STAGE_TRY(map_staging(host_pinned, &stg, "shg_stage_extract"));
    const char* end = dense ? reinterpret_cast<const char*>(h_base + ih) : reinterpret_cast<const char*>(h_w2 + 2 * ih);
    if (minmax_slots) {
        const size_t n_words = ((size_t)(end - reinterpret_cast<const char*>(h_ind)) + 3) / 4, zero_words = (size_t)n_shifts * 130;
        const unsigned blocks = (unsigned)std::min<size_t>((std::max(n_words, zero_words) + 255) / 256, 64);
        STAGE_TRY(shg::launch(k_words_zero, dim3(blocks), dim3(256), 0, st,
                             WordsArgs{reinterpret_cast<uint32_t*>(ind_l), reinterpret_cast<const uint32_t*>(stg.on_device(h_ind)), n_words, minmax_slots, zero_words}, "k_words_zero"));
        shg::t_minmax_slots_zeroed = true;
    } else {
        STAGE_TRY(move_words(ind_l, stg.on_device(h_ind), (size_t)(end - reinterpret_cast<const char*>(h_ind)), st));
    }
    if (dense)
        return shg_extract_columns_dense(stack, n_frames, height, width, bytes_per_px, frame_stride_px, ind_l, base, w2, w2 + ih, host_shifts, n_shifts,
                                         disks, row_pitch, plane_stride, n_cols, k_offset, flip_x, minmax_slots, stream);
    return shg_extract_columns_minmax(stack, n_frames, height, width, bytes_per_px, frame_stride_px, ind_l, w2, w2 + ih, n_shifts, disks,
                                      row_pitch, plane_stride, n_cols, k_offset, flip_x, minmax_slots, stream);
}

namespace {
constexpr int kFactor = 4;
inline int64_t small_dim(int64_t v) { return (v + kFactor - 1) / kFactor; }

inline bool limb_fused(int64_t sh, int64_t sw, int k) {
    const char* v = getenv("SHG_LIMB_FUSED");
    return !(v && v[0] == '0') && k > 0 && shg_limb_fused_fits(sh, sw, k);
}

int64_t keep_strong_components(int32_t* idx, int32_t* root, int64_t m, int64_t n) {
    thread_local std::vector<uint8_t> strong;
    if ((int64_t)strong.size() < n) strong.assign((size_t)n, 0);
    for (int64_t i = 0; i < m; ++i)
        if (root[i] & (1 << 30)) strong[(size_t)(root[i] & 0x3fffffff)] = 1;
    int64_t kept = 0;
    for (int64_t i = 0; i < m; ++i) {
        const int32_t r = root[i] & 0x3fffffff;
        if (strong[(size_t)r]) { idx[kept] = idx[i]; root[kept] = r; ++kept; }
    }
    for (int64_t i = 0; i < kept; ++i) strong[(size_t)root[i]] = 0;
    return kept;
}
}

extern "C" size_t shg_stage_limb_points_workspace_bytes(int64_t h, int64_t w) {
    if (h <= 0 || w <= 0) return 0;
    const int64_t sh = small_dim(h), sw = small_dim(w);
    const size_t n = (size_t)sh * (size_t)sw;
    const int k = (int)((double)sh * 0.01);
    if (limb_fused(sh, sw, k)) return up(shg_limb_prepare_workspace_bytes(sh, sw, k)) + up(shg_limb_edges_workspace_bytes(sh, sw)) + kAlign;
    return 4 * up(n * 8) + up(std::max(shg_select_workspace_bytes(4), shg_select_keys_workspace_bytes(4))) + 2 * up(n * 4) + up(4 * 8) + up(3 * 8) + up(20 * 4) + up(256) + up(32 * 8) + 2 * up(n) +
           up(shg_canny_workspace_bytes(sh, sw)) + up(shg_edge_components_workspace_bytes(sh, sw)) + up((2 * n + 1) * 4) + kAlign;
}

extern "C" size_t shg_stage_limb_points_host_bytes(int64_t h, int64_t w) {
    if (h <= 0 || w <= 0) return 0;
    const size_t n = (size_t)small_dim(h) * (size_t)small_dim(w);
    return up(32 * 8) + up((2 * n + 1) * 4);
}

extern "C" int shg_stage_limb_points(const uint16_t* disk, int64_t h, int64_t w, int64_t pitch, const double* host_gauss_taps,
                                     int32_t* host_points, uint8_t* host_flags, int64_t points_cap, int64_t* host_counts2,
                                     void* workspace, size_t workspace_bytes, void* host_pinned, size_t host_pinned_bytes,
                                     shg_stream_t stream) {
    SHG_REQUIRE(disk && host_gauss_taps && host_points && host_flags && host_counts2 && workspace && host_pinned, SHG_E_ARG,
                "shg_stage_limb_points: null pointer");
    SHG_REQUIRE(h > 0 && w > 0 && pitch >= w, SHG_E_ARG, "shg_stage_limb_points: bad image size");
    const int64_t sh = small_dim(h), sw = small_dim(w);
    const int64_t n = sh * sw;
    const int k = (int)((double)sh * 0.01);
    if (k <= 0) {
        shg::set_error("ellipse fit: the scan needs at least 400 slit rows (cv2.blur kernel int(0.01 * h/4) = 0)");
        return SHG_E_RUNTIME;
    }
    hipStream_t st = shg::as_stream(stream);
    if (limb_fused(sh, sw, k)) {
        Arena dev(workspace, workspace_bytes), pin(host_pinned, host_pinned_bytes);
        const size_t prep_bytes = shg_limb_prepare_workspace_bytes(sh, sw, k), edge_bytes = shg_limb_edges_workspace_bytes(sh, sw);
        char* prep_ws = dev.take<char>(prep_bytes);
        char* edge_ws = dev.take<char>(edge_bytes);
        double* h_packed = pin.take<double>(32);
        int32_t* h_comp = pin.take<int32_t>(2 * (size_t)n + 1);
        SHG_REQUIRE(prep_ws && edge_ws, SHG_E_WORKSPACE, "shg_stage_limb_points: workspace too small");
        SHG_REQUIRE(h_packed && h_comp, SHG_E_WORKSPACE, "shg_stage_limb_points: pinned staging area too small");
        Staging stg;
        STAGE_TRY(map_staging(host_pinned, &stg, "shg_stage_limb_points"));
        int64_t ranks[4];
        double gamma99;
        ranks[0] = (n & 1) ? n / 2 : n / 2 - 1;
        ranks[1] = n / 2;
        STAGE_TRY(shg_host_percentile_plan(n, 99.0, &ranks[2], &ranks[3], &gamma99));
        const uint32_t* keys = nullptr;
        STAGE_TRY(shg_limb_prepare(disk, h, w, pitch, k, ranks, gamma99, stg.on_device(h_packed), &keys, prep_ws, prep_bytes, stream));
// ... 68 lines not shown
        STAGE_TRY(shg_box_blur_key_f64(small, sh, sw, k, blurred, keys_k, tmp, stream));
        if (k == 5) {
            blur5 = blurred;
            keys_5 = keys_k;
        } else {
            STAGE_TRY(shg_box_blur_key_f64(small, sh, sw, 5, blur5, keys_5, tmp, stream));
        }
        const uint32_t* karr[4] = {keys_5, keys_5, keys_k, keys_k};
        const int kk[4] = {5, 5, k, k};
        STAGE_TRY(shg_select_keys_u32(karr, n, ranks, kk, 4, packed, sel_ws, sel_bytes, stream));
    } else {
        STAGE_TRY(shg_box_blur_f64(small, sh, sw, k, blurred, tmp, stream));
        STAGE_TRY(shg_box_blur_f64(small, sh, sw, 5, blur5, tmp, stream));
        const double* arrays[4] = {blur5, blur5, blurred, blurred};
        STAGE_TRY(shg_select_multi_f64(arrays, n, ranks, 4, packed, sel_ws, sel_bytes, stream));
    }
    STAGE_TRY(shg_flood_stats_lerp_f64(small, blurred, n, packed + 2, gamma99, packed + 4, counts, flood_ws, stream));
    STAGE_TRY(move_words(stg.on_device(h_packed), packed, 8 * 8 + 20 * 4, st));
    STAGE_SYNC(st, "shg_stage_limb_points");
    const double median5 = (n & 1) ? h_packed[0] : (h_packed[0] + h_packed[1]) / 2;
    const double low = median5 / 10, high = low * 1.5;
    int64_t counts64[20];
    const uint32_t* hc = reinterpret_cast<const uint32_t*>(h_packed + 8);
    for (int i = 0; i < 20; ++i) counts64[i] = hc[i];
    double thresh3;
    STAGE_TRY(shg_host_flood_threshold(h_packed[4], sh, sw, h_packed[5], h_packed[6], counts64, &thresh3));

    int64_t m = 0;
    const double* taps = host_gauss_taps;
    for (int rung = 0;; ++rung) {
        if (rung == 4) { shg::set_error("ellipse fit: could not find any edges of the solar disk"); return SHG_E_RUNTIME; }
        const double sigma = 2.0 - 0.5 * rung;
        const int radius = (int)(4.0 * sigma + 0.5);
        STAGE_TRY(shg_canny_masks_f64(blurred, sh, sw, thresh3, taps, radius, low, high, low_mask, high_mask, canny_ws, canny_bytes, stream));
        STAGE_TRY(shg_edge_components(low_mask, high_mask, sh, sw, comp + 1, comp + 1 + n, comp, cc_ws, cc_bytes, stream));
        k_edge_list<<<16, 256, 0, st>>>(comp, n, stg.on_device(h_comp));
        STAGE_TRY(shg::check_launch("k_edge_list"));
        STAGE_SYNC(st, "shg_stage_limb_points");
        m = h_comp[0];
        SHG_REQUIRE(m >= 0 && m <= n, SHG_E_RUNTIME, "shg_stage_limb_points: %lld edge pixels in an image of %lld", (long long)m, (long long)n);
        if (m > 0) break;
        taps += 2 * radius + 1;
    }
    const int32_t* idx = h_comp + 1;
    const int32_t* root = h_comp + 1 + n;
    SHG_REQUIRE(points_cap >= m, SHG_E_WORKSPACE, "shg_stage_limb_points: %lld edge pixels, room for %lld", (long long)m, (long long)points_cap);
    int64_t n_sel = 0;
    STAGE_TRY(shg_host_limb_points(idx, root, m, sh, sw, host_flags, &n_sel));
    for (int64_t i = 0; i < m; ++i) {
        host_points[2 * i] = idx[i] / (int32_t)sw;
        host_points[2 * i + 1] = idx[i] % (int32_t)sw;
    }
    host_counts2[0] = m;
    host_counts2[1] = n_sel;
    return 0;
}

extern "C" int shg_stage_limb_fit(const uint16_t* disk, int64_t h, int64_t w, int64_t pitch, const double* host_gauss_taps,
                                  int32_t* host_points, uint8_t* host_flags, int64_t points_cap, int64_t* host_counts3,
                                  double* host_geom16, int64_t* host_dims2, double* host_outline200, void* workspace,
                                  size_t workspace_bytes, void* host_pinned, size_t host_pinned_bytes, shg_stream_t stream) {
    SHG_HOST_TIME("stage limb_fit");
    SHG_REQUIRE(host_counts3 && host_geom16 && host_dims2, SHG_E_ARG, "shg_stage_limb_fit: null pointer");
    STAGE_TRY(shg_stage_limb_points(disk, h, w, pitch, host_gauss_taps, host_points, host_flags, points_cap, host_counts3, workspace,
                                    workspace_bytes, host_pinned, host_pinned_bytes, stream));
    const int64_t m = host_counts3[0], n_sel = host_counts3[1];
    std::vector<double> X((size_t)std::max<int64_t>(n_sel, 1) * 2);
    std::vector<uint8_t> kept((size_t)std::max<int64_t>(n_sel, 1));
    for (int64_t i = 0, j = 0; i < m; ++i)
        if (host_flags[i]) {
            X[2 * j] = (double)host_points[2 * i] * kFactor;
            X[2 * j + 1] = (double)host_points[2 * i + 1] * kFactor;
            ++j;
        }
    STAGE_TRY(shg_host_limb_geometry(X.data(), n_sel, h, w, host_geom16, host_dims2, kept.data(), &host_counts3[2], host_outline200));
    for (int64_t i = 0, j = 0; i < m; ++i)
        if (host_flags[i]) { if (kept[j]) host_flags[i] |= 2; ++j; }
    return 0;
}

extern "C" size_t shg_stage_process_workspace_bytes(int64_t k, int64_t h, int64_t w, int64_t crop_w, int tiles) {
    if (k <= 0 || h <= 0 || w <= 0) return 0;
    const size_t pitch = ((size_t)std::max(w, crop_w) + 63) / 64 * 64;
    return 2 * up((size_t)h * 4) + 2 * up((size_t)k * h * 8) + up((size_t)k * h * 8) + up(4096 * 8) +
           (size_t)k * up((size_t)h * pitch * 2) + (size_t)k * up(shg_contrast_stats_workspace_bytes_for(h, crop_w > 0 ? crop_w : w, tiles)) + up((size_t)k * 5 * 8) + kAlign;
}

extern "C" size_t shg_stage_process_host_bytes(int64_t k, int64_t h) {
    if (k <= 0 || h <= 0) return 0;
    return 2 * up((size_t)h * 4) + 2 * up((size_t)k * h * 8) + up((size_t)k * h * 8) + up((size_t)k * 5 * 8) + up(4096 * 8);
}

extern "C" int shg_stage_process_frames(const uint16_t* const* host_frames, int64_t k, int64_t h, int64_t w, int64_t pitch,
                                        int transversalium, const double* host_circle3, const double* host_borders4,
                                        const double* host_taps, int64_t window, double* host_factors,
                                        int64_t crop_w, int64_t sx0, int64_t dx0, int64_t ncopy,
                                        double clip_limit, int tiles, int64_t disc_x0, int64_t disc_y0, int64_t disc_r,
                                        uint16_t* const* host_detrans, int64_t detrans_pitch,
                                        uint16_t* const* host_final, uint16_t* const* host_cl1, uint16_t* const* host_hc,
                                        uint16_t* const* host_protus, uint16_t* const* host_cc, int64_t out_pitch,
                                        void* workspace, size_t workspace_bytes, void* host_pinned, size_t host_pinned_bytes,
                                        shg_stream_t stream) {
    SHG_HOST_TIME("stage process_frames");
    SHG_REQUIRE(host_frames && host_final && host_cl1 && host_hc && host_protus && host_cc && workspace && host_pinned, SHG_E_ARG,
                "shg_stage_process_frames: null pointer");
    SHG_REQUIRE(k > 0 && h > 0 && w > 0 && pitch >= w, SHG_E_ARG, "shg_stage_process_frames: bad image size");
    const int64_t out_w = crop_w > 0 ? crop_w : w;
    SHG_REQUIRE(out_pitch >= out_w, SHG_E_ARG, "shg_stage_process_frames: out_pitch < output width");
    hipStream_t st = shg::as_stream(stream);
    Arena dev(workspace, workspace_bytes), pin(host_pinned, host_pinned_bytes);
    int32_t* xa = dev.take<int32_t>((size_t)h);
    int32_t* xb = dev.take<int32_t>((size_t)h);
    double* taps_d = dev.take<double>(4096);
    double* stats = dev.take<double>((size_t)k * h);
    double* interior = dev.take<double>((size_t)k * h);
    double* factors = dev.take<double>((size_t)k * h);
    const size_t tpitch = ((size_t)w + 63) / 64 * 64;
    std::vector<uint16_t*> scaled((size_t)k, nullptr);
    const char* fuse_env = getenv("SHG_FUSE_SCALE");
    const bool fuse_on = !(fuse_env && fuse_env[0] == '0');
    const bool fuse = fuse_on && !host_detrans && shg::contrast_stats_batches(h, crop_w > 0 ? crop_w : w, tiles, clip_limit) && pitch >= w;
    const bool need_tmp = transversalium && crop_w > 0 && !host_detrans && !fuse;
    if (need_tmp)
        for (int64_t i = 0; i < k; ++i) scaled[i] = dev.take<uint16_t>((size_t)h * tpitch);
    const size_t cs_each = up(shg_contrast_stats_workspace_bytes_for(h, out_w, tiles));
    SHG_REQUIRE(cs_each != 0, SHG_E_ARG, "shg_stage_process_frames: unsupported tile count %d", tiles);
    const size_t cs_bytes = (size_t)k * cs_each;
    char* cs_ws = dev.take<char>(cs_bytes);
    double* out5 = dev.take<double>((size_t)k * 5);
    int32_t* h_xa = pin.take<int32_t>((size_t)h);
    int32_t* h_xb = pin.take<int32_t>((size_t)h);
    double* h_taps = pin.take<double>(4096);
    double* h_stats = pin.take<double>((size_t)k * h);
    double* h_interior = pin.take<double>((size_t)k * h);
    double* h_factors = pin.take<double>((size_t)k * h);
    double* h_out5 = pin.take<double>((size_t)k * 5);
    SHG_REQUIRE(xa && xb && stats && interior && factors && taps_d && cs_ws && out5 && (!need_tmp || scaled[k - 1]), SHG_E_WORKSPACE,
                "shg_stage_process_frames: workspace too small");
    SHG_REQUIRE(h_xa && h_xb && h_stats && h_interior && h_factors && h_out5 && h_taps, SHG_E_WORKSPACE, "shg_stage_process_frames: pinned staging area too small");
    Staging stg;
    STAGE_TRY(map_staging(host_pinned, &stg, "shg_stage_process_frames"));

    std::vector<const uint16_t*> cur((size_t)k);
    int64_t cur_pitch = pitch;
    for (int64_t i = 0; i < k; ++i) cur[i] = host_frames[i];
    if (transversalium) {
        SHG_REQUIRE(host_circle3 && host_borders4 && host_taps, SHG_E_ARG, "shg_stage_process_frames: transversalium needs circle, borders, taps");
        const double cx = host_circle3[0], cy = host_circle3[1], r = host_circle3[2];
        const int64_t y1 = (int64_t)ceil(std::max(cy - r, host_borders4[1])), y2 = (int64_t)floor(std::min(cy + r, host_borders4[3]));
        int64_t n = 1;
        bool have_rows = y2 - y1 >= 1;
        const double* use_interior = nullptr;
        if (have_rows) {
            SHG_REQUIRE(y1 >= 0 && y2 <= h, SHG_E_ARG, "shg_stage_process_frames: rows [%lld, %lld) outside the image", (long long)y1, (long long)y2);
            n = y2 - y1;
            STAGE_TRY(shg_host_chord_bounds(cx, cy, r, host_borders4[0], host_borders4[2], y1, y2, w, h_xa, h_xb));
            const bool gpu_interior = window > 3 && window <= n && window / 2 <= 1024 && window <= 4096;
            std::vector<double> rev;
            if (gpu_interior) {
                rev.resize((size_t)window);
                for (int64_t i = 0; i < window; ++i) rev[i] = host_taps[window - 1 - i];
                memcpy(h_taps, rev.data(), (size_t)window * 8);
            }
            const char* plan_end = gpu_interior ? reinterpret_cast<const char*>(h_taps + window) : reinterpret_cast<const char*>(h_xb + n);
            STAGE_TRY(move_words(xa, stg.on_device(h_xa), (size_t)(plan_end - reinterpret_cast<const char*>(h_xa)), st));
            STAGE_TRY(shg::rowpair_stats_batch(host_frames, k, h, w, pitch, y1, y2, xa, xb, nullptr, stats, stg.on_device(h_stats), stream));
            if (gpu_interior) {
                const int radius = (int)(window / 2);
                int sym = 1, anti = 1;
                for (int i = 1; i <= radius; ++i) {
                    if (fabs(rev[radius + i] - rev[radius - i]) > 2.220446049250313e-16) sym = 0;
                    if (fabs(rev[radius + i] + rev[radius - i]) > 2.220446049250313e-16) anti = 0;
                }
                STAGE_TRY(shg_correlate1d_rows_f64(stats, k, n, taps_d, radius, sym ? 1 : (anti ? -1 : 0), stg.on_device(h_interior), stream));
                use_interior = h_interior;
            }
            STAGE_SYNC(st, "shg_stage_process_frames");
        } else {
            for (int64_t i = 0; i < k; ++i) h_stats[i] = 0.0;
        }
        std::vector<double> corr((size_t)k * n);
        STAGE_TRY(shg_host_transversalium_factors(h_stats, use_interior, k, n, host_taps, window, 1, corr.data()));
        for (int64_t i = 0; i < k; ++i) {
            double* c = h_factors + i * h;
            for (int64_t y = 0; y < h; ++y) c[y] = 1.0;
            if (have_rows) memcpy(c + y1, corr.data() + i * n, (size_t)n * 8);
        }
        if (host_factors) memcpy(host_factors, h_factors, (size_t)k * h * 8);
        factors = stg.on_device(h_factors);
      if (!fuse) {
        std::vector<uint16_t*> dsts((size_t)k);
        int64_t dpitch = out_pitch;
        for (int64_t i = 0; i < k; ++i) {
            if (host_detrans) { dsts[i] = host_detrans[i]; dpitch = detrans_pitch; }
            else if (crop_w > 0) { dsts[i] = scaled[i]; dpitch = (int64_t)tpitch; }
            else { dsts[i] = host_final[i]; dpitch = out_pitch; }
            SHG_REQUIRE(dsts[i] && dpitch >= w, SHG_E_ARG, "shg_stage_process_frames: bad de-transversalium output");
            cur[i] = dsts[i];
        }
        cur_pitch = dpitch;
        STAGE_TRY(shg::scale_rows_batch(host_frames, k, h, w, pitch, factors, nullptr, dsts.data(), dpitch, stream));
      }
    }
    if (fuse) {
    } else if (crop_w > 0) {
        STAGE_TRY(shg::crop_pad_batch(cur.data(), k, h, w, cur_pitch, host_final, crop_w, out_pitch, sx0, dx0, ncopy, -1, stream));
    } else if (cur[0] != host_final[0]) {
        STAGE_TRY(shg::crop_pad_batch(cur.data(), k, h, w, cur_pitch, host_final, w, out_pitch, 0, 0, w, -1, stream));
    }
    const int64_t n_px = h * out_w;
    int64_t ranks_frame[2], ranks_cl1[3];
    double g_bright, g_dark;
    STAGE_TRY(shg_host_percentile_plan(n_px, 99.9999, &ranks_frame[0], &ranks_frame[1], &g_bright));
    STAGE_TRY(shg_host_percentile_plan(n_px, 10.0, &ranks_cl1[0], &ranks_cl1[1], &g_dark));
    ranks_cl1[2] = n_px - 1;
    shg::FrameSource from = {host_frames, pitch, transversalium ? factors : nullptr, crop_w > 0 ? sx0 : 0, crop_w > 0 ? dx0 : 0, crop_w > 0 ? ncopy : w};
    STAGE_TRY(shg::contrast_stats_batch(host_final, k, h, out_w, out_pitch, clip_limit, tiles, host_cl1, out_pitch, ranks_frame, ranks_cl1, out5, cs_ws,
                                        cs_bytes, stream, fuse ? &from : nullptr));
    STAGE_TRY(shg::contrast_products_batch(host_final, out_pitch, host_cl1, out_pitch, k, h, out_w, nullptr, host_hc, host_protus, host_cc, out_pitch,
                                           disc_x0, disc_y0, disc_r, stream, out5, g_bright, g_dark, stg.on_device(h_out5)));
    STAGE_SYNC(st, "shg_stage_process_frames");
    bool again = false;
    for (int64_t i = 0; i < k; ++i) {
        const double* s = h_out5 + i * 5;
        if (s[0] == s[0] && s[1] == s[1]) continue;
        again = true;
        SHG_HOST_TIME("frame percentile selected over the image");
        STAGE_TRY(shg_select_u16(host_final[i], h, out_w, out_pitch, ranks_frame, 2, out5 + 5 * i, cs_ws + (size_t)i * cs_each, cs_each, stream));
        STAGE_TRY(shg::contrast_products_batch(host_final + i, out_pitch, host_cl1 + i, out_pitch, 1, h, out_w, nullptr, host_hc + i, host_protus + i, host_cc + i,
                                               out_pitch, disc_x0, disc_y0, disc_r, stream, out5 + 5 * i, g_bright, g_dark, stg.on_device(h_out5 + 5 * i)));
    }
    if (again) STAGE_SYNC(st, "shg_stage_process_frames");
    for (int64_t i = 0; i < k; ++i) {
        const double* s = h_out5 + i * 5;
        const double bright = shg_host_lerp(s[0], s[1], g_bright);
        const double dark_clahe = shg_host_lerp(s[2], s[3], g_dark);
        const double bright_clahe = (double)(int64_t)s[4];
        if (!(65535 >= bright && bright > bright * 0.25 && 65535 >= bright * 0.18 && bright * 0.18 > 0 && 65535 >= bright_clahe &&
              bright_clahe > dark_clahe)) {
            shg::set_error("rescale_brightness: assert sat >= hi > lo (bright %g, clahe %g .. %g)", bright, dark_clahe, bright_clahe);
            return SHG_E_ASSERT;
        }
    }
    return 0;
}
```

### solex_ser_recon_en_amd/csrc/transversalium.hip

```cpp
#include <math.h>
#include <algorithm>
#include "shg_common.h"
#include "fast_log.h"

namespace {

constexpr int MAXN = SHG_TRANSV_MAX_COLS;
constexpr int NT = 256;

__device__ __forceinline__ uint64_t f64_key(double v) {
    const uint64_t b = (uint64_t)__double_as_longlong(v);
    return (b >> 63) ? ~b : (b | 0x8000000000000000ull);
}
__device__ __forceinline__ double key_f64(uint64_t k) {
    const uint64_t b = (k >> 63) ? (k & 0x7fffffffffffffffull) : ~k;
    return __longlong_as_double((long long)b);
}

constexpr int NB = 512;
constexpr int CAP = 128;

struct alignas(16) Scratch {
    uint32_t hist[2][256];
    int64_t wave_tot[2][4];
// ... 447 lines not shown
    const int64_t x = (int64_t)blockIdx.x * 256 + threadIdx.x;
    const int64_t y = blockIdx.y;
    if (x >= w) return;
    const uint16_t* __restrict__ img = imgs.at<const uint16_t>(blockIdx.z);
    uint16_t* __restrict__ dst = dsts.at<uint16_t>(blockIdx.z);
    c += (int64_t)blockIdx.z * gridDim.y;
    double v = (double)img[y * pitch + x];
    if (row_factor) v = v * row_factor[y];
    v = v * c[y];
    v = v > 65535.0 ? 65535.0 : v;
    dst[y * dst_pitch + x] = (uint16_t)(int)v;
}

constexpr int SCALE_ROWS = 4;
__global__ __launch_bounds__(256) void k_scale_rows8(shg::PtrBatch imgs, int64_t h, int64_t w, int64_t pitch,
                                                     const double* __restrict__ c, const double* __restrict__ row_factor,
                                                     shg::PtrBatch dsts, int64_t dst_pitch) {
    const uint32_t nv = (uint32_t)((w + 7) / 8);
    const uint32_t flat = blockIdx.x * 256u + threadIdx.x;
    const uint32_t yg = flat / nv;
    const int64_t x = (int64_t)(flat - yg * nv) * 8;
    const int64_t ya = (int64_t)yg * SCALE_ROWS;
    if (ya >= h) return;
    const uint16_t* __restrict__ img = imgs.at<const uint16_t>(blockIdx.z);
    uint16_t* __restrict__ dst = dsts.at<uint16_t>(blockIdx.z);
    c += (int64_t)blockIdx.z * h;
    const bool factored = row_factor != nullptr;
    const bool full = x + 8 <= w;
    uint4 q[SCALE_ROWS];
    double cy[SCALE_ROWS], fy[SCALE_ROWS];
#pragma unroll
    for (int rr = 0; rr < SCALE_ROWS; ++rr) {
        const int64_t y = ya + rr < h ? ya + rr : h - 1;
        if (full) q[rr] = *reinterpret_cast<const uint4*>(img + y * pitch + x);
        cy[rr] = c[y];
        fy[rr] = factored ? row_factor[y] : 1.0;
    }
#pragma unroll
    for (int rr = 0; rr < SCALE_ROWS; ++rr) {
        const int64_t y = ya + rr;
        if (y >= h) break;
        const double cyr = cy[rr], fyr = fy[rr];
        auto one = [&](uint32_t px) {
            double v = (double)px;
            if (factored) v = v * fyr;
            v = v * cyr;
            v = v > 65535.0 ? 65535.0 : v;
            return (uint32_t)(int)v;
        };
        if (full) {
            uint4 o;
            o.x = one(q[rr].x & 0xffffu) | (one(q[rr].x >> 16) << 16);
            o.y = one(q[rr].y & 0xffffu) | (one(q[rr].y >> 16) << 16);
            o.z = one(q[rr].z & 0xffffu) | (one(q[rr].z >> 16) << 16);
            o.w = one(q[rr].w & 0xffffu) | (one(q[rr].w >> 16) << 16);
            *reinterpret_cast<uint4*>(dst + y * dst_pitch + x) = o;
        } else {
            for (int64_t i = x; i < w; ++i) dst[y * dst_pitch + i] = (uint16_t)one(img[y * pitch + i]);
        }
    }
}

constexpr int CORR_MAXR = 1024;

struct CorrelateArgs {
    const double* src;
    int64_t n;
    const double* weights;
    int radius, symmetric;
    double* dst;
};

__global__ __launch_bounds__(256) void k_correlate1d_rows(const CorrelateArgs kargs) {
    const double* __restrict__ src = kargs.src;
    const int64_t n = kargs.n;
    const double* __restrict__ weights = kargs.weights;
    const int radius = kargs.radius, symmetric = kargs.symmetric;
    double* __restrict__ dst = kargs.dst;
    extern __shared__ double corr_lds[];
    double* xs = corr_lds;
    double* ws = corr_lds + 256 + 2 * radius;
    const int64_t row = blockIdx.y, x0 = (int64_t)blockIdx.x * 256;
    const double* line = src + row * n;
    for (int i = threadIdx.x; i < 256 + 2 * radius; i += 256) {
        const int64_t xx = x0 - radius + i;
        xs[i] = (xx >= 0 && xx < n) ? line[xx] : 0.0;
    }
    for (int i = threadIdx.x; i < 2 * radius + 1; i += 256) ws[i] = weights[i];
    __syncthreads();
    const int64_t x = x0 + threadIdx.x;
    if (x >= n) return;
    const double* c = xs + radius + threadIdx.x;
    const double* w = ws + radius;
    double t;
    if (symmetric > 0) {
        t = c[0] * w[0];
        for (int j = -radius; j < 0; ++j) t += (c[j] + c[-j]) * w[j];
    } else if (symmetric < 0) {
        t = c[0] * w[0];
        for (int j = -radius; j < 0; ++j) t += (c[j] - c[-j]) * w[j];
    } else {
        t = c[radius] * w[radius];
        for (int j = -radius; j < radius; ++j) t += c[j] * w[j];
    }
    dst[row * n + x] = t;
}

__global__ __launch_bounds__(NT) void k_line_order_stats(const uint16_t* __restrict__ img, int64_t pitch, int n, int64_t line_stride,
                                                         int64_t elem_stride, int rank_lo, int rank_hi,
                                                         uint16_t* __restrict__ out_lo, uint16_t* __restrict__ out_hi) {
    __shared__ uint32_t hist[256];
    __shared__ int pick[2][2];
    const uint16_t* line = img + (int64_t)blockIdx.x * line_stride;
    int rank[2] = {rank_lo, rank_hi};
    int hi_digit[2] = {0, 0};
    int result[2] = {0, 0};
    for (int pass = 0; pass < 3; ++pass) {
        if (pass == 2 && hi_digit[0] == hi_digit[1]) break;
        const int which = pass == 2 ? 1 : 0;
        hist[threadIdx.x] = 0;
        __syncthreads();
        for (int i = threadIdx.x; i < n; i += NT) {
            const uint32_t v = line[(int64_t)i * elem_stride];
            if (pass == 0) atomicAdd(&hist[v >> 8], 1u);
            else if ((int)(v >> 8) == hi_digit[which]) atomicAdd(&hist[v & 0xff], 1u);
        }
        __syncthreads();
        if (threadIdx.x == 0) {
            for (int r = 0; r < 2; ++r) {
                if (pass == 2 && r == 0) continue;
                if (pass == 1 && r == 1 && hi_digit[1] != hi_digit[0]) continue;
                int below = 0, d = 0;
                for (; d < 256; ++d) {
                    const int c = (int)hist[d];
                    if (below + c > rank[r]) break;
                    below += c;
                }
                pick[r][0] = d;
                pick[r][1] = below;
            }
        }
        __syncthreads();
        for (int r = 0; r < 2; ++r) {
            if (pass == 2 && r == 0) continue;
            if (pass == 1 && r == 1 && hi_digit[1] != hi_digit[0]) continue;
            if (pass == 0) { hi_digit[r] = pick[r][0]; rank[r] -= pick[r][1]; }
            else result[r] = (hi_digit[r] << 8) | pick[r][0];
        }
        __syncthreads();
    }
    if (threadIdx.x == 0) {
        out_lo[blockIdx.x] = (uint16_t)result[0];
        out_hi[blockIdx.x] = (uint16_t)result[1];
    }
}

}

extern "C" int shg_line_order_stats_u16(const uint16_t* img, int64_t h, int64_t w, int64_t pitch, int axis, int64_t rank_lo,
                                        int64_t rank_hi, uint16_t* out_lo, uint16_t* out_hi, shg_stream_t stream) {
    SHG_REQUIRE(img && out_lo && out_hi, SHG_E_ARG, "shg_line_order_stats_u16: null pointer");
    SHG_REQUIRE(h > 0 && w > 0 && pitch >= w && (axis == 0 || axis == 1), SHG_E_ARG, "shg_line_order_stats_u16: bad arguments");
    const int64_t n = axis == 0 ? h : w, lines = axis == 0 ? w : h;
    SHG_REQUIRE(n < (1ll << 31) && rank_lo >= 0 && rank_lo <= rank_hi && rank_hi < n, SHG_E_ARG,
                "shg_line_order_stats_u16: ranks [%lld, %lld] outside a line of %lld", (long long)rank_lo, (long long)rank_hi, (long long)n);
    hipStream_t st = shg::as_stream(stream);
    SHG_PROF("line_order_stats", st);
    k_line_order_stats<<<(unsigned)lines, NT, 0, st>>>(img, pitch, (int)n, axis == 0 ? 1 : pitch, axis == 0 ? pitch : 1, (int)rank_lo,
                                                      (int)rank_hi, out_lo, out_hi);
    return shg::check_launch("k_line_order_stats");
}
// ... 97 lines not shown
```

### solex_ser_recon_en_amd/csrc/warp.hip

```cpp
#include <algorithm>
#include <cmath>
#include "shg_common.h"
#include <type_traits>

namespace {

__global__ void k_minmax_init(uint32_t* mm) {
    mm[0] = 0xffffffffu;
    mm[1] = 0u;
}

__global__ __launch_bounds__(256) void k_minmax(const uint16_t* __restrict__ src, int64_t h, int64_t w, int64_t pitch,
                                                uint32_t* __restrict__ mm) {
    uint32_t lo = 0xffffffffu, hi = 0u;
    for (int64_t y0 = blockIdx.x; y0 < h; y0 += 8 * (int64_t)gridDim.x) {
        for (int64_t x = threadIdx.x; x < w; x += 256) {
            uint32_t v[8];
            bool ok[8];
#pragma unroll
            for (int u = 0; u < 8; ++u) {
                const int64_t y = y0 + u * (int64_t)gridDim.x;
                ok[u] = y < h;
                v[u] = src[(ok[u] ? y : y0) * pitch + x];
            }
#pragma unroll
            for (int u = 0; u < 8; ++u) {
                if (ok[u]) {
                    lo = v[u] < lo ? v[u] : lo;
                    hi = v[u] > hi ? v[u] : hi;
                }
            }
        }
    }
#pragma unroll
    for (int d = 32; d >= 1; d >>= 1) {
        const uint32_t ol = __shfl_xor(lo, d), oh = __shfl_xor(hi, d);
        lo = ol < lo ? ol : lo;
        hi = oh > hi ? oh : hi;
    }
    __shared__ uint32_t wlo[4], whi[4];
    if ((threadIdx.x & 63) == 0) { wlo[threadIdx.x >> 6] = lo; whi[threadIdx.x >> 6] = hi; }
    __syncthreads();
    if (threadIdx.x == 0) {
        for (int i = 1; i < 4; ++i) { lo = wlo[i] < lo ? wlo[i] : lo; hi = whi[i] > hi ? whi[i] : hi; }
        atomicMin(&mm[0], lo);
        atomicMax(&mm[1], hi);
    }
}

constexpr int kWarpBatch = 24;
struct WarpRows { double h[kWarpBatch][3]; };

using WarpPtrs = shg::PtrBatchN<kWarpBatch>;
struct WarpArgs {
    WarpPtrs srcs;
    int64_t h, w, pitch;
    WarpRows rows;
    WarpPtrs dsts;
    int64_t out_h, out_w, dst_pitch;
    WarpPtrs mms;
    uint32_t nv_magic, nv_shift;
};

template <int WARP_ROWS>
__global__ __launch_bounds__(256) void k_warp_rows(const WarpArgs kargs) {
    const WarpPtrs& srcs = kargs.srcs;
    const WarpPtrs& dsts = kargs.dsts;
    const WarpPtrs& mms = kargs.mms;
    const int64_t h = kargs.h, w = kargs.w, pitch = kargs.pitch, out_h = kargs.out_h, out_w = kargs.out_w, dst_pitch = kargs.dst_pitch;
    const WarpRows& rows = kargs.rows;
    const uint16_t* __restrict__ src = srcs.at<const uint16_t>(blockIdx.z);
    uint16_t* __restrict__ dst = dsts.at<uint16_t>(blockIdx.z);
    const uint32_t* __restrict__ mm = mms.at<const uint32_t>(blockIdx.z);
    const double h00 = rows.h[blockIdx.z][0], h01 = rows.h[blockIdx.z][1], h02 = rows.h[blockIdx.z][2];
    const int c = (int)(blockIdx.x * 256 + threadIdx.x);
    const int ra = (int)blockIdx.y * WARP_ROWS;
    if (c >= out_w) return;
    double dc[WARP_ROWS];
    uint32_t v0[WARP_ROWS], v1[WARP_ROWS];
    bool in0[WARP_ROWS], in1[WARP_ROWS];
    const bool sane = fabs(h00) < 1e300 && fabs(h01) < 1e300 && fabs(h02) < 1e300;
    const uint32_t wu = (uint32_t)w;
    const double xc = h00 * (double)c;
#pragma unroll
    for (int rr = 0; rr < WARP_ROWS; ++rr) {
        const int r = ra + rr;
        const double x = xc + h01 * (double)r + h02;
        const double x0 = floor(x);
        dc[rr] = x - x0;
        const int i0 = __double2int_rz(x0);
        const int i1 = dc[rr] != 0.0 ? (i0 == 0x7fffffff ? i0 : i0 + 1) : i0;
        const bool row_ok = sane && r < h;
        in0[rr] = row_ok && (uint32_t)i0 < wu;
        in1[rr] = row_ok && (uint32_t)i1 < wu;
        const uint16_t* row = src + (int64_t)(row_ok ? r : 0) * pitch;
        v0[rr] = row[in0[rr] ? i0 : 0];
        v1[rr] = row[in1[rr] ? i1 : 0];
    }
    const uint32_t cval = src[0];
    const double lo = (double)mm[0], hi = (double)mm[1];
#pragma unroll
    for (int rr = 0; rr < WARP_ROWS; ++rr) {
        const int r = ra + rr;
        if (r >= out_h) break;
        const double left = (double)(in0[rr] ? v0[rr] : cval), right = (double)(in1[rr] ? v1[rr] : cval);
        double v = (1.0 - dc[rr]) * left + dc[rr] * right;
        v = fmin(fmax(v, lo), hi);
        dst[(int64_t)r * dst_pitch + c] = (uint16_t)(int)v;
    }
}

typedef unsigned int __attribute__((ext_vector_type(4))) u32x4_t;
typedef unsigned int __attribute__((ext_vector_type(3))) u32x3_t;
constexpr int kWarpPairs = 22;
template <int ITER>
__global__ __launch_bounds__(256) __attribute__((amdgpu_waves_per_eu(7))) void k_warp_rows8(const WarpArgs kargs) {
    __shared__ uint32_t win[4][kWarpPairs][64];
    const int64_t h = kargs.h, w = kargs.w, pitch = kargs.pitch, out_h = kargs.out_h, out_w = kargs.out_w, dst_pitch = kargs.dst_pitch;
    const uint16_t* __restrict__ src = kargs.srcs.at<const uint16_t>(blockIdx.z);
    uint16_t* __restrict__ dst = kargs.dsts.at<uint16_t>(blockIdx.z);
    const uint32_t* __restrict__ mm = kargs.mms.at<const uint32_t>(blockIdx.z);
    const double h00 = kargs.rows.h[blockIdx.z][0], h01 = kargs.rows.h[blockIdx.z][1], h02 = kargs.rows.h[blockIdx.z][2];
    const uint32_t nv = (uint32_t)((out_w + 7) / 8), total = nv * (uint32_t)out_h;
    const int lane = threadIdx.x & 63, wave = threadIdx.x >> 6;
    uint32_t (*const my)[64] = win[wave];
    const uint32_t cval = src[0];
    const int lo_i = (int)mm[0], hi_i = (int)mm[1];
    const double k00 = h00 * 0x1p+52;
    const uint32_t wu = (uint32_t)w;
    const int w_last = (int)w - 1, last_piece = (int)pitch - 8;

    auto place = [&](int it, int& r, int& c, int& ws, double& hr, double& x) {
        const uint32_t flat = ((uint32_t)blockIdx.x * ITER + (uint32_t)it) * 256u + threadIdx.x;
        const uint32_t f = flat < total ? flat : total - 1;
        r = (int)(__umulhi(f, kargs.nv_magic) >> kargs.nv_shift);
        c = (int)(f - (uint32_t)r * nv) * 8;
        hr = h01 * (double)r;
        x = h00 * (double)c + hr + h02;
        const int i0 = __double2int_rz(floor(x));
        ws = min(max(i0, 0), w_last) & ~7;
        return flat < total;
    };
    const char* const src_bytes = reinterpret_cast<const char*>(src);
    const uint32_t pitch_u = (uint32_t)pitch, dst_pitch_u = (uint32_t)dst_pitch, hu = (uint32_t)h;
    auto fetch = [&](int r, int ws, u32x4_t (&q)[2], u32x3_t& q2) {
        const uint32_t row = __umul24((uint32_t)r < hu ? (uint32_t)r : 0u, pitch_u);
#pragma unroll
        for (int t = 0; t < 2; ++t) q[t] = *reinterpret_cast<const u32x4_t*>(src_bytes + ((row + (uint32_t)min(ws + 8 * t, last_piece)) << 1));
        q2 = *reinterpret_cast<const u32x3_t*>(src_bytes + ((row + (uint32_t)min(ws + 16, last_piece)) << 1));
    };
    int r, c, ws;
    double hr_next, x_next;
    bool live = place(0, r, c, ws, hr_next, x_next);
    u32x4_t q[2];
    u32x3_t q2;
    fetch(r, ws, q, q2);
#pragma unroll 1
    for (int it = 0; it < ITER; ++it) {
        if (!__any(live)) break;
        {
            const uint32_t wd[11] = {q[0].x, q[0].y, q[0].z, q[0].w, q[1].x, q[1].y, q[1].z, q[1].w, q2.x, q2.y, q2.z};
            my[0][lane] = wd[0] << 16;
#pragma unroll
            for (int k = 0; k < 11; ++k) my[1 + 2 * k][lane] = wd[k];
#pragma unroll
            for (int k = 0; k < 10; ++k) my[2 + 2 * k][lane] = __builtin_amdgcn_alignbit(wd[k + 1], wd[k], 16);
        }
        const int r_now = r, c_now = c, ws_now = ws;
        const double hr = hr_next, x_first = x_next;
        const bool live_now = live;
        if (it + 1 < ITER) {
            live = place(it + 1, r, c, ws, hr_next, x_next);
            fetch(r, ws, q, q2);
        }
        const uint32_t w_row = r_now < h ? wu : 0u;
        const int ws1 = ws_now - 1;
        const double col0 = __hiloint2double(0x43300000, c_now);
        uint32_t out[8];
        auto pixels = [&](auto inside_tag) {
            constexpr bool INSIDE = decltype(inside_tag)::value;
#pragma unroll
            for (int j = 0; j < 8; ++j) {
                const double x = j == 0 ? x_first : __builtin_fma(col0 + (double)j, h00, -k00) + hr + h02;
                const double x0 = floor(x);
                const double dc = x - x0;
                const int i0 = __double2int_rz(x0);
                const int row = INSIDE ? i0 - ws1 : min(max(i0 - ws1, 0), kWarpPairs - 1);
                const uint32_t pair = *reinterpret_cast<const uint32_t*>(reinterpret_cast<const char*>(&my[0][lane]) + ((uint32_t)row << 8));
                double left, right;
                if constexpr (INSIDE) {
                    left = (double)(pair & 0xffffu);
                    right = (double)(pair >> 16);
                } else {
                    const bool in0 = (uint32_t)i0 < w_row, in1 = (uint32_t)i0 + 1u < w_row;
                    left = (double)(in0 ? (pair & 0xffffu) : cval);
                    right = (double)(in1 ? pair >> 16 : cval);
                }
                const double v = (1.0 - dc) * left + dc * right;
                out[j] = (uint32_t)min(max((int)v, lo_i), hi_i);
            }
        };
        const double x_last = __builtin_fma(col0 + 7.0, h00, -k00) + hr + h02;
        const bool inside = x_first >= 0.0 && x_last < (double)w_last && r_now < h;
        if (__all(inside)) pixels(std::true_type{});
        else pixels(std::false_type{});
        if (live_now) {
            uint16_t* o = reinterpret_cast<uint16_t*>(reinterpret_cast<char*>(dst) + ((__umul24((uint32_t)r_now, dst_pitch_u) + (uint32_t)c_now) << 1));
            if (c_now + 8 <= out_w) {
                const u32x4_t pk = {out[0] | (out[1] << 16), out[2] | (out[3] << 16), out[4] | (out[5] << 16), out[6] | (out[7] << 16)};
                *reinterpret_cast<u32x4_t*>(o) = pk;
            } else {
#pragma unroll
                for (int j = 0; j < 8; ++j)
                    if (c_now + j < out_w) o[j] = (uint16_t)out[j];
            }
        }
    }
}

constexpr int64_t kWarpWideAbove = 16384;
int warp_rows_forced() {
    static const int v = [] { const char* e = getenv("SHG_WARP_ROWS"); const int n = e ? atoi(e) : 0; return n == 4 || n == 8 || n == 16 ? n : 0; }();
    return v;
}

}

extern "C" int shg_warp_rows_u16(const uint16_t* src, int64_t h, int64_t w, int64_t src_pitch, double h00, double h01,
                                 double h02, uint16_t* dst, int64_t out_h, int64_t out_w, int64_t dst_pitch,
                                 uint32_t* minmax, shg_stream_t stream) {
    SHG_REQUIRE(src && dst && minmax, SHG_E_ARG, "shg_warp_rows_u16: null pointer");
    SHG_REQUIRE(h > 0 && w > 0 && out_h > 0 && out_w > 0, SHG_E_ARG, "shg_warp_rows_u16: empty image");
    SHG_REQUIRE(src_pitch >= w && dst_pitch >= out_w, SHG_E_ARG, "shg_warp_rows_u16: pitch smaller than width");
    SHG_REQUIRE(out_h < 65536, SHG_E_UNSUPPORTED, "shg_warp_rows_u16: more than 65535 rows");
    hipStream_t st = shg::as_stream(stream);
    { SHG_PROF("minmax", st); k_minmax_init<<<1, 1, 0, st>>>(minmax); }
    int64_t blocks = h < 256 ? h : 256;
    { SHG_PROF("minmax", st); k_minmax<<<(unsigned)blocks, 256, 0, st>>>(src, h, w, src_pitch, minmax); }
    if (int e = shg::check_launch("k_minmax")) return e;
    const double h3[3] = {h00, h01, h02};
    const uint32_t* mm = minmax;
    return shg::warp_rows_batch(&src, 1, h, w, src_pitch, h3, &dst, out_h, out_w, dst_pitch, &mm, stream);
}

extern "C" int shg_warp_rows_minmax_u16(const uint16_t* src, int64_t h, int64_t w, int64_t src_pitch, double h00, double h01,
                                        double h02, uint16_t* dst, int64_t out_h, int64_t out_w, int64_t dst_pitch,
                                        const uint32_t* minmax2, shg_stream_t stream) {
    SHG_REQUIRE(src && dst && minmax2, SHG_E_ARG, "shg_warp_rows_minmax_u16: null pointer");
    const double h3[3] = {h00, h01, h02};
    return shg::warp_rows_batch(&src, 1, h, w, src_pitch, h3, &dst, out_h, out_w, dst_pitch, &minmax2, stream);
}

int shg::warp_rows_batch(const uint16_t* const* host_srcs, int64_t k, int64_t h, int64_t w, int64_t src_pitch, const double* host_h3,
                         uint16_t* const* host_dsts, int64_t out_h, int64_t out_w, int64_t dst_pitch, const uint32_t* const* host_minmax2,
                         shg_stream_t stream) {
    SHG_REQUIRE(host_srcs && host_h3 && host_dsts && host_minmax2 && k > 0, SHG_E_ARG, "shg_warp_rows_minmax_u16: null pointer");
    SHG_REQUIRE(h > 0 && w > 0 && out_h > 0 && out_w > 0, SHG_E_ARG, "shg_warp_rows_minmax_u16: empty image");
    SHG_REQUIRE(src_pitch >= w && dst_pitch >= out_w, SHG_E_ARG, "shg_warp_rows_minmax_u16: pitch smaller than width");
    SHG_REQUIRE(out_h < 65536 && out_w < (1ll << 30) && w < (1ll << 30) && h < (1ll << 30), SHG_E_UNSUPPORTED, "shg_warp_rows_minmax_u16: image too large");
    for (int64_t i = 0; i < k; ++i) SHG_REQUIRE(host_srcs[i] && host_dsts[i] && host_minmax2[i], SHG_E_ARG, "shg_warp_rows_minmax_u16: null image");
    hipStream_t st = shg::as_stream(stream);
    SHG_PROF("warp", st);
    for (int64_t i0 = 0; i0 < k; i0 += kWarpBatch) {
        const int m = (int)std::min<int64_t>(kWarpBatch, k - i0);
        WarpRows rows = {};
        for (int d = 0; d < m; ++d)
            for (int j = 0; j < 3; ++j) rows.h[d][j] = host_h3[3 * (i0 + d) + j];
        const uint64_t nv = (uint64_t)((out_w + 7) / 8);
        uint32_t nv_shift = 0;
        while ((2ull << nv_shift) < nv) ++nv_shift;
        const uint32_t nv_magic = nv >= 2 ? (uint32_t)(((1ull << (32 + nv_shift)) + nv - 1) / nv) : 0u;
        const WarpArgs args{shg::make_batch_n<kWarpBatch>(host_srcs, (int)i0, m), h, w, src_pitch, rows, shg::make_batch_n<kWarpBatch>(host_dsts, (int)i0, m),
                            out_h, out_w, dst_pitch, shg::make_batch_n<kWarpBatch>(host_minmax2, (int)i0, m), nv_magic, nv_shift};
        const bool wide_ok = [] { const char* e = getenv("SHG_WARP_WIDE"); return !e || atoi(e) != 0; }();
        bool wide = wide_ok && src_pitch % 8 == 0 && dst_pitch % 8 == 0 && w >= 8 && src_pitch >= 8 && nv >= 2 && out_h * ((out_w + 7) / 8) < (1ll << 31) &&
                    src_pitch < (1ll << 24) && dst_pitch < (1ll << 24) && h * src_pitch < (1ll << 31) && out_h * dst_pitch < (1ll << 31);
        for (int d = 0; d < m && wide; ++d) {
            const double a00 = rows.h[d][0], a01 = rows.h[d][1], a02 = rows.h[d][2];
            wide = a00 >= 0.0 && a00 <= 1.75 && std::fabs(a01) < 1e300 && std::fabs(a02) < 1e300 &&
                   (reinterpret_cast<uintptr_t>(host_srcs[i0 + d]) & 15) == 0 && (reinterpret_cast<uintptr_t>(host_dsts[i0 + d]) & 15) == 0;
        }
        if (wide) {
            const int64_t vecs = out_h * ((out_w + 7) / 8);
            const bool few = vecs * m < 4 * 256 * 2048;
            auto go8 = [&](auto I) {
                dim3 grid((unsigned)((vecs + 256 * I.value - 1) / (256 * I.value)), 1u, (unsigned)m);
                return shg::launch(k_warp_rows8<I.value>, grid, dim3(256), 0, st, args, "k_warp_rows8");
            };
            if (int e = few ? go8(std::integral_constant<int, 1>{}) : go8(std::integral_constant<int, 4>{})) return e;
            continue;
        }
        const int64_t gx = (out_w + 255) / 256;
        int rows_per_lane = gx * ((out_h + 7) / 8) * m >= kWarpWideAbove ? 8 : 4;
        if (warp_rows_forced()) rows_per_lane = warp_rows_forced();
        auto go = [&](auto R) {
            dim3 grid((unsigned)gx, (unsigned)((out_h + R.value - 1) / R.value), (unsigned)m);
            return shg::launch(k_warp_rows<R.value>, grid, dim3(256), 0, st, args, "k_warp_rows");
        };
        const int e = rows_per_lane == 16 ? go(std::integral_constant<int, 16>{})
                    : rows_per_lane == 8 ? go(std::integral_constant<int, 8>{}) : go(std::integral_constant<int, 4>{});
        if (e) return e;
    }
    return 0;
}
```

### solex_ser_recon_en_amd/stages.py

```python
import ctypes
import os
import threading

import numpy as np
import torch

from . import _lib, ops
from ._lib import lib

_local = threading.local()


def use_buffers(store):
    _local.buffers = store


def _scratch(name, nbytes, device=None, pinned=False):
    store = _local.__dict__.setdefault('buffers', {})
    key = (name, str(device), pinned)
    buf = store.get(key)
    if buf is None or buf.numel() < nbytes:
        size = max(int(nbytes), 1)
        if pinned:
            buf = torch.empty(size, dtype=torch.uint8).pin_memory()
# ... 358 lines not shown
        pin_bytes = _sizes('scan_pin', lambda *a: lib.shg_scan_host_bytes(ctypes.byref(rq)), s, k, n, h, w, bpp, limb)
        self.pin = _lease_pinned(pin_bytes) if own_buffers else _scratch('scan', pin_bytes, pinned=True)
        self.rs = _lib.ScanResult()
        self.status = None
        self.message = None
        self.pool = self.ticket = None
        self._buffers()

    def _buffers(self):
        rq, hint, dev = self.rq, self.hint, self.dev
        self.arena = arena = torch.empty(_even256(hint[0]), dtype=torch.uint8, device=dev)
        self.results = results = torch.empty(_even256(hint[1]), dtype=torch.uint8, device=dev)
        self.ws = ws = torch.empty(_even256(hint[2]), dtype=torch.uint8, device=dev) if self.own else _scratch('scan', hint[2], dev)
        rq.arena, rq.arena_bytes, rq.results, rq.results_bytes = arena.data_ptr(), arena.numel(), results.data_ptr(), results.numel()
        rq.workspace, rq.workspace_bytes = ws.data_ptr(), ws.numel()
        rq.host_pinned, rq.host_pinned_bytes = self.pin.data_ptr(), self.pin.numel()

    def _needs_resume(self):
        rs = self.rs
        if self.status == -2 and rs.phase_done == 3 and self.rq.start_phase == 0:
            self.hint = (rs.needed_arena_bytes + 4096, rs.needed_results_bytes + 4096, rs.needed_workspace_bytes + 4096)
            self.rq.start_phase = 3
            self._buffers()
            return True
        return False

    def run(self):
        stream = ops._stream()
        while True:
            self.status = lib.shg_scan_file(ctypes.byref(self.rq), ctypes.byref(self.rs), stream)
            self.message = _lib.last_error() if self.status else None
            if not self._needs_resume():
                return self

    def submit(self, pool):
        self.pool = pool
        ticket = ctypes.c_int64()
        after = torch.cuda.current_stream(self.stack.device).cuda_stream
        _lib.check(lib.shg_pool_submit_after(pool, ctypes.byref(self.rq), ctypes.byref(self.rs), after, ctypes.byref(ticket)),
                   'shg_pool_submit')
        self.ticket = ticket.value
        return self

    def done(self):
        return self.ticket is None or lib.shg_pool_poll(self.pool, self.ticket) != 0

    def wait(self):
        while self.ticket is not None:
            status = ctypes.c_int()
            buf = ctypes.create_string_buffer(512)
            _lib.check(lib.shg_pool_wait(self.pool, self.ticket, ctypes.byref(status), buf, len(buf)), 'shg_pool_wait')
            self.ticket = None
            self.status = status.value
            self.message = buf.value.decode('utf-8', 'replace') if self.status else None
            if self._needs_resume():
                self.submit(self.pool)
        return self

    def collect(self):
        rs, rq = self.rs, self.rq
        s, k, n = self.s, self.k, self.n
        phase = int(rs.phase_done)
        if (phase >= 3 and _arena_hint.get(self.key) is None) or rq.start_phase == 3:
            _arena_hint[self.key] = (int(rs.needed_arena_bytes * 1.03) + 4096, int(rs.needed_results_bytes * 1.03) + 4096,
                                     int(rs.needed_workspace_bytes * 1.03) + 4096)
        error = None
        if self.status != 0:
            error = _lib.take_callback_error(rs.window)
            if error is None:
                try:
                    _lib.check(self.status, 'shg_scan_file', self.message)
                except Exception as e:
                    error = e
        out = {'phase': phase, 'mean': self.images[0], 'max': self.images[1], 'limb_fitted': bool(rs.limb_fitted)}
        if phase >= 1:
            y1, y2 = int(rs.y1), int(rs.y2)
            out['y1'], out['y2'], out['p'] = y1, y2, np.array(rs.p4)
            if self.plot:
                out['fit'] = self.fit.copy()
                out['sharp'] = self.sharp.copy()
                out['mask_good'] = self.mask[:max(y2 - y1, 0)].astype(bool)
        if phase >= 2:
            out['disks'] = self.disks[:, :, :n]
            out['extrema'] = self.mm_store[s * 128:].view(s, 2)
        if phase >= 3:
            out['phi'], out['ratio'] = float(rs.phi), float(rs.ratio)
            out['theta_first'] = float(rs.theta_first)
            out['circle'] = (rs.circle3[0], rs.circle3[1], rs.circle3[2])
            out['borders'] = list(rs.borders4)
            if rs.limb_fitted and self.plot:
                m = int(rs.counts3[0])
                pts, fl = self.points[:m].astype(np.int64) * 4, self.flags[:m]
                out['raw_X'], out['X_f'], out['outline'] = pts, pts[(fl & 2) != 0].astype(float), self.outline.copy()
        if phase >= 4:
            oh, ow, fp, pw, pp = int(rs.out_h), int(rs.out_w), int(rs.frame_pitch), int(rs.prod_w), int(rs.prod_pitch)
            fb = (oh * fp * 2 + 255) // 256 * 256
            pb = (oh * pp * 2 + 255) // 256 * 256
            ap, rp = _Planes(self.arena), _Planes(self.results)
            out['fit_image'] = ap.plane(int(rs.fit_image_off), oh, fp, ow) if rs.fit_image_off >= 0 else None
            out['frames'] = _LazyImages(ap, int(rs.frames_off), fb, k, oh, fp, ow)
            out['detrans'] = _LazyImages(ap, int(rs.detrans_off), fb, k, oh, fp, ow) if rs.detrans_off >= 0 else None
            for idx, name in enumerate(('final', 'cl1', 'hc')):
                out[name] = _LazyImages(ap, int(rs.products_off) + idx * pb, 3 * pb, k, oh, pp, pw)
            for idx, name in enumerate(('protus', 'cc')):
                out[name] = _LazyImages(rp, idx * pb, 2 * pb, k, oh, pp, pw)
            out['factors'] = self.factors[:k].copy() if (self.trans and k) else None
        if self.own:
            _return_pinned(self.pin)
            _return_host(self.specs, self.bufs)
            self.pin = self.bufs = self.fit = self.sharp = self.mask = self.points = self.flags = self.outline = self.factors = None
        return out, error


def scan_file(stack, shifts, requested, options, taps_for, want_plot_data=False, want_fit_image=False):
    return ScanCall(stack, shifts, requested, options, taps_for, want_plot_data, want_fit_image).run().collect()
```

Baseline: 6.164 million.

## Fold extrema in warp kernel, fuse limb histogram into blur, drop staging copies

Result: slower. 6.100 million (-1.0%).

```diff
diff --git a/solex_ser_recon_en_amd/Solex_recon.py b/solex_ser_recon_en_amd/Solex_recon.py
--- a/solex_ser_recon_en_amd/Solex_recon.py
+++ b/solex_ser_recon_en_amd/Solex_recon.py
@@ -604,7 +604,7 @@
         if phase >= 2:
             hdr['NAXIS1'] = rdr.iw
             if options['save_fit'] or plots or (phase >= 3 and not r['limb_fitted'] and requested[0] and '_nolog' not in options):
-                disk_list = [DeviceImage(r['disks'][i], minmax=r['extrema'][i]) for i in range(len(shifts))]
+                disk_list = [DeviceImage(r['disks'][i]) for i in range(len(shifts))]
             if options.get('_keep_raw'):
                 options['_raw_disks'] = [DeviceImage(r['disks'][i]) for i in range(len(shifts))]
             for i, disk in enumerate(disk_list):
diff --git a/solex_ser_recon_en_amd/csrc/extract.hip b/solex_ser_recon_en_amd/csrc/extract.hip
--- a/solex_ser_recon_en_amd/csrc/extract.hip
+++ b/solex_ser_recon_en_amd/csrc/extract.hip
@@ -5,9 +5,10 @@
 
 namespace shg {
 thread_local bool t_minmax_slots_zeroed = false;
-thread_local void* t_zero_with_fold = nullptr;
-thread_local size_t t_zero_with_fold_words = 0;
+thread_local void* t_zero_with_plan = nullptr;
+thread_local size_t t_zero_with_plan_words = 0;
 thread_local void* t_prezeroed = nullptr;
+thread_local bool t_extrema_read_from_slots = false;
 }
 
 namespace {
@@ -530,39 +531,20 @@
 struct FoldMinmaxArgs {
     const uint32_t* slots;
     uint32_t* out;
-    int n_planes;
-    uint32_t* zero;
-    size_t zero_words;
 };
 
 __global__ __launch_bounds__(64) void k_fold_minmax(const FoldMinmaxArgs kargs) {
     const uint32_t* __restrict__ slots = kargs.slots;
     uint32_t* __restrict__ out = kargs.out;
-    if ((int)blockIdx.x >= kargs.n_planes) {
-        uint32_t* __restrict__ z = kargs.zero;
-        const size_t stride = (size_t)(gridDim.x - kargs.n_planes) * 64;
-        for (size_t i = (size_t)(blockIdx.x - kargs.n_planes) * 64 + threadIdx.x; i < kargs.zero_words; i += stride) z[i] = 0;
-        return;
-    }
     uint32_t a = slots[((int64_t)blockIdx.x * 64 + threadIdx.x) * 2], b = slots[((int64_t)blockIdx.x * 64 + threadIdx.x) * 2 + 1];
     a = shg::wave_fold_u32(a, [](uint32_t x, uint32_t y) { return x > y ? x : y; });
     b = shg::wave_fold_u32(b, [](uint32_t x, uint32_t y) { return x > y ? x : y; });
     if (threadIdx.x == 0) { out[blockIdx.x * 2] = 0xffffu - a; out[blockIdx.x * 2 + 1] = b; }
 }
 
-int launch_fold(uint32_t* minmax_slots, int n_shifts, hipStream_t st) {
-    FoldMinmaxArgs fa{minmax_slots, minmax_slots + (int64_t)n_shifts * 64 * 2, n_shifts, nullptr, 0};
-    unsigned extra = 0;
-    if (shg::t_zero_with_fold && shg::t_zero_with_fold_words > 0) {
-        fa.zero = static_cast<uint32_t*>(shg::t_zero_with_fold);
-        fa.zero_words = shg::t_zero_with_fold_words;
-        extra = (unsigned)std::min<size_t>((fa.zero_words + 1023) / 1024, 64);
-    }
-    const int e = shg::launch(k_fold_minmax, dim3((unsigned)n_shifts + extra), dim3(64), 0, st, fa, "k_fold_minmax");
-    if (e == 0 && extra) shg::t_prezeroed = shg::t_zero_with_fold;
-    shg::t_zero_with_fold = nullptr;
-    shg::t_zero_with_fold_words = 0;
-    return e;
+int launch_fold(uint32_t* minmax_slots, int n_shifts, bool reader_folds, hipStream_t st) {
+    if (reader_folds) return 0;
+    return shg::launch(k_fold_minmax, dim3((unsigned)n_shifts), dim3(64), 0, st, FoldMinmaxArgs{minmax_slots, minmax_slots + (int64_t)n_shifts * 64 * 2}, "k_fold_minmax");
 }
 
 }
@@ -581,6 +563,8 @@
                                           int64_t n_cols, int64_t k_offset, int flip_x, uint32_t* minmax_slots, shg_stream_t stream) {
     const bool slots_zeroed = shg::t_minmax_slots_zeroed;
     shg::t_minmax_slots_zeroed = false;
+    const bool reader_folds = shg::t_extrema_read_from_slots;
+    shg::t_extrema_read_from_slots = false;
     SHG_REQUIRE(stack && ind_l && lw && rw && disks, SHG_E_ARG, "shg_extract_columns: null pointer");
     SHG_REQUIRE(n_frames > 0 && height > 0 && width > 0 && n_shifts > 0, SHG_E_ARG, "shg_extract_columns: empty input");
     SHG_REQUIRE(bytes_per_px == 1 || bytes_per_px == 2, SHG_E_ARG, "shg_extract_columns: bytes_per_px must be 1 or 2");
@@ -629,7 +613,7 @@
                     minmax_slots, (int)((n_cols + TK - 1) / TK), {}};
         launch_status = launch_band<false>(ba, bytes_per_px, ih, st);
         if (launch_status) return launch_status;
-        if (minmax_slots) return launch_fold(minmax_slots, n_shifts, st);
+        if (minmax_slots) return launch_fold(minmax_slots, n_shifts, reader_folds, st);
         return 0;
     }
     if (bytes_per_px == 2) {
@@ -641,7 +625,7 @@
 #undef EXT_LAUNCH_BS
 #undef EXT_LAUNCH
     if (launch_status) return launch_status;
-    if (minmax_slots) return launch_fold(minmax_slots, n_shifts, st);
+    if (minmax_slots) return launch_fold(minmax_slots, n_shifts, reader_folds, st);
     return 0;
 }
 
@@ -665,6 +649,8 @@
                                          shg_stream_t stream) {
     const bool slots_zeroed = shg::t_minmax_slots_zeroed;
     shg::t_minmax_slots_zeroed = false;
+    const bool reader_folds = shg::t_extrema_read_from_slots;
+    shg::t_extrema_read_from_slots = false;
     SHG_REQUIRE(stack && ind_l && base_col && lw && rw && host_shifts && disks, SHG_E_ARG, "shg_extract_columns_dense: null pointer");
     SHG_REQUIRE(n_frames > 0 && height > 0 && width > 0, SHG_E_ARG, "shg_extract_columns_dense: empty input");
     SHG_REQUIRE(shg_extract_dense_fits(host_shifts, n_shifts), SHG_E_UNSUPPORTED, "shg_extract_columns_dense: the shifts are not 3..%d consecutive integers", DS_MAX);
@@ -696,7 +682,7 @@
         for (int i = 0; i < n_shifts; ++i) ba.plane_of[host_shifts[i] - lo] = (uint8_t)i;
         const int launch_status = launch_band<true>(ba, bytes_per_px, ih, st);
         if (launch_status) return launch_status;
-        if (minmax_slots) return launch_fold(minmax_slots, n_shifts, st);
+        if (minmax_slots) return launch_fold(minmax_slots, n_shifts, reader_folds, st);
         return 0;
     }
     static const int shape = [] { const char* e = getenv("SHG_EXT_DENSE_SHAPE"); return e ? atoi(e) : 0; }();
@@ -729,6 +715,6 @@
 #undef SHG_DENSE_S
 #undef SHG_DENSE
     if (launch_status) return launch_status;
-    if (minmax_slots) return launch_fold(minmax_slots, n_shifts, st);
+    if (minmax_slots) return launch_fold(minmax_slots, n_shifts, reader_folds, st);
     return 0;
 }
diff --git a/solex_ser_recon_en_amd/csrc/limb_fused.hip b/solex_ser_recon_en_amd/csrc/limb_fused.hip
--- a/solex_ser_recon_en_amd/csrc/limb_fused.hip
+++ b/solex_ser_recon_en_amd/csrc/limb_fused.hip
@@ -115,6 +115,8 @@
     int sh, sw, k, vec4;
     uint32_t *keysk, *keys5;
     unsigned long long* acc;
+    int bits0, bits1;
+    uint32_t *hist0, *coarse0;
 };
 __global__ __launch_bounds__(256) void k_limb_blur(const LimbBlurArgs kargs) {
     const uint16_t* __restrict__ img = kargs.img;
@@ -127,6 +129,9 @@
     __shared__ uint32_t H[(BT + KMAX) * BT];
     __shared__ unsigned long long wsum[4];
     __shared__ uint32_t wmin[4];
+    extern __shared__ uint32_t lds[];
+    __shared__ uint32_t lc[256];
+    const int bits0 = kargs.bits0, bits1 = kargs.bits1;
     const int hl = max(k / 2, 2), hr = max(k - 1 - k / 2, 2);
     const int RH = BT + hl + hr, RW = RH;
     const int x0 = blockIdx.x * BT, y0 = blockIdx.y * BT;
@@ -163,6 +168,7 @@
     for (int a = 0; a < n_arrays; ++a) {
         const int kw = a == 0 ? k : 5;
         uint32_t* keys = a == 0 ? keysk : keys5;
+        for (int e = tid; e < (1 << bits0); e += 256) lds[e] = 0;
         __syncthreads();
         const int c_off = hl - kw / 2, r_lo = hl - kw / 2, r_n = BT + kw - 1;
         for (int e = tid; e < r_n * BT; e += 256) {
@@ -178,7 +184,10 @@
             for (int j = 0; j < kw; ++j) s += H[(r_lo + y + j) * BT + x];
             keys[(int64_t)(y0 + y) * sw + x0 + x] = s;
             if (a == 0) my_min = s;
-        }
+            atomicAdd(&lds[s >> bits1], 1u);
+        }
+        __syncthreads();
+        flush_hist(lds, bits0, lc, kargs.hist0 + ((size_t)a << bits0), kargs.coarse0 + a * 256, tid, 256);
     }
     my_min = shg::wave_fold_u32(my_min, [](uint32_t x, uint32_t y) { return x < y ? x : y; });
     if ((tid & 63) == 0) wmin[tid >> 6] = my_min;
@@ -228,39 +237,6 @@
 }
 
 struct Ranks4 { int64_t rank[4]; int array[4]; double scale[4]; };
-
-struct LimbSelect0Args {
-    const uint32_t *keysk, *keys5;
-    int64_t n;
-    int bits0, bits1;
-    uint32_t *hist0, *coarse0;
-};
-__global__ __launch_bounds__(256) void k_limb_select0(const LimbSelect0Args kargs) {
-    const uint32_t* __restrict__ keysk = kargs.keysk;
-    const uint32_t* __restrict__ keys5 = kargs.keys5;
-    const int64_t n = kargs.n;
-    const int bits0 = kargs.bits0, bits1 = kargs.bits1;
-    uint32_t* __restrict__ hist0 = kargs.hist0;
-    uint32_t* __restrict__ coarse0 = kargs.coarse0;
-    extern __shared__ uint32_t lds[];
-    __shared__ uint32_t lc[256];
-    const int a = blockIdx.y;
-    const uint32_t* __restrict__ v = a ? keys5 : keysk;
-    for (int e = threadIdx.x; e < (1 << bits0); e += 256) lds[e] = 0;
-    __syncthreads();
-    const int64_t stride = (int64_t)gridDim.x * 256;
-    for (int64_t base = (int64_t)blockIdx.x * 256 + threadIdx.x; base < n; base += 4 * stride) {
-        uint32_t kk[4];
-        bool ok[4];
-#pragma unroll
-        for (int u = 0; u < 4; ++u) { const int64_t i = base + u * stride; ok[u] = i < n; kk[u] = v[ok[u] ? i : 0]; }
-#pragma unroll
-        for (int u = 0; u < 4; ++u)
-            if (ok[u]) atomicAdd(&lds[kk[u] >> bits1], 1u);
-    }
-    __syncthreads();
-    flush_hist(lds, bits0, lc, hist0 + ((size_t)a << bits0), coarse0 + a * 256, threadIdx.x, 256);
-}
 
 struct LimbSelect1Args {
     const uint32_t *keysk, *keys5;
@@ -778,17 +754,16 @@
     for (int i = 0; i < 4; ++i) { p.rank[i] = host_ranks4[i]; p.array[i] = (i < 2 && k != 5) ? 1 : 0; p.scale[i] = (i < 2) ? scale_5 : scale_k; }
     dim3 grid1((unsigned)((sw + BT - 1) / BT), (unsigned)((sh + BT - 1) / BT));
     const int vec4 = (reinterpret_cast<uintptr_t>(img) & 7) == 0 && pitch % 4 == 0;
-    if (int e = shg::launch(k_limb_blur, grid1, dim3(256), 0, st, LimbBlurArgs{img, (int)h, (int)w, pitch, (int)sh, (int)sw, k, vec4, keysk, keys5, acc}, "k_limb_blur")) return e;
     static const bool lds_ok = [] {
-        return hipFuncSetAttribute(reinterpret_cast<const void*>(k_limb_select0), hipFuncAttributeMaxDynamicSharedMemorySize, 128 * 1024) == hipSuccess &&
+        return hipFuncSetAttribute(reinterpret_cast<const void*>(k_limb_blur), hipFuncAttributeMaxDynamicSharedMemorySize, 128 * 1024) == hipSuccess &&
                hipFuncSetAttribute(reinterpret_cast<const void*>(k_limb_select1), hipFuncAttributeMaxDynamicSharedMemorySize, 128 * 1024) == hipSuccess;
     }();
     if (!lds_ok) (void)hipGetLastError();
+    if (int e = shg::launch(k_limb_blur, grid1, dim3(256), ((size_t)1 << lay.bits0) * 4, st,
+                           LimbBlurArgs{img, (int)h, (int)w, pitch, (int)sh, (int)sw, k, vec4, keysk, keys5, acc, lay.bits0, lay.bits1, hist0, coarse0}, "k_limb_blur"))
+        return e;
     int64_t blocks = (n + 2047) / 2048;
     if (blocks > 256) blocks = 256;
-    if (int e = shg::launch(k_limb_select0, dim3((unsigned)blocks, k == 5 ? 1u : 2u), dim3(256), ((size_t)1 << lay.bits0) * 4, st,
-                           LimbSelect0Args{keysk, keys5, n, lay.bits0, lay.bits1, hist0, coarse0}, "k_limb_select0"))
-        return e;
     if (int e = shg::launch(k_limb_select1, dim3((unsigned)blocks, 4u), dim3(256), ((size_t)1 << lay.bits1) * 4, st,
                            LimbSelect1Args{keysk, keys5, n, p, lay.bits0, lay.bits1, hist0, coarse0, hist1, coarse1, gamma99, done, acc, out4, limb_fence()}, "k_limb_select1"))
         return e;
diff --git a/solex_ser_recon_en_amd/csrc/scan.hip b/solex_ser_recon_en_amd/csrc/scan.hip
--- a/solex_ser_recon_en_amd/csrc/scan.hip
+++ b/solex_ser_recon_en_amd/csrc/scan.hip
@@ -196,14 +196,16 @@
         rs->y2 = y12[1];
         rs->phase_done = 1;
         if (limb) {
-            shg::t_zero_with_fold = limb_ws;
-            shg::t_zero_with_fold_words = shg::limb_prepare_zero_words(ih, n_cols);
+            shg::t_zero_with_plan = limb_ws;
+            shg::t_zero_with_plan_words = shg::limb_prepare_zero_words(ih, n_cols);
         }
+        shg::t_extrema_read_from_slots = true;
         const int extract_status = shg_stage_extract(rq->stack, rq->n_frames, rq->height, rq->width, rq->bytes_per_px, rq->frame_stride_px, rq->host_fit,
                                                      rq->host_shifts, S, rq->disks, rq->disk_pitch, rq->disk_plane_stride, n_cols, 0, rq->flip_x,
                                                      rq->minmax_slots, extract_ws, rg.extract_ws, extract_pin, rg.extract_pin, stream);
-        shg::t_zero_with_fold = nullptr;
-        shg::t_zero_with_fold_words = 0;
+        shg::t_zero_with_plan = nullptr;
+        shg::t_zero_with_plan_words = 0;
+        shg::t_extrema_read_from_slots = false;
         if (extract_status) { shg::t_prezeroed = nullptr; return extract_status; }
         rs->phase_done = 2;
         bool later_disks = false;
@@ -287,7 +289,6 @@
                 "shg_scan_file: arenas not 256-byte aligned");
     char* arena = static_cast<char*>(rq->arena);
     char* results = static_cast<char*>(rq->results);
-    const uint32_t* extrema = rq->minmax_slots + (size_t)S * 128;
     std::vector<const uint16_t*> w_src;
     std::vector<uint16_t*> w_dst;
     std::vector<const uint32_t*> w_mm;
@@ -296,7 +297,7 @@
         const double* hr = i == 0 ? rs->h_first : rs->h_rest;
         w_src.push_back(rq->disks + (size_t)i * rq->disk_plane_stride);
         w_dst.push_back(dst);
-        w_mm.push_back(extrema + 2 * i);
+        w_mm.push_back(rq->minmax_slots + (size_t)i * 128);
         w_h.insert(w_h.end(), hr, hr + 3);
     };
     if (fit_image) add_warp(0, reinterpret_cast<uint16_t*>(arena + rs->fit_image_off));
@@ -316,7 +317,7 @@
     }
     if (!w_src.empty())
         SCAN_TRY(shg::warp_rows_batch(w_src.data(), (int64_t)w_src.size(), ih, n_cols, rq->disk_pitch, w_h.data(), w_dst.data(), out_h, out_w, frame_pitch,
-                                      w_mm.data(), stream));
+                                      w_mm.data(), stream, true));
     if (k > 0) {
         SCAN_TRY(shg_stage_process_frames(frames.data(), k, out_h, out_w, frame_pitch, rq->transversalium, pl.trans_circle, pl.trans_borders,
                                           pl.taps_ptr, pl.window, rq->host_factors, pl.crop_w, pl.sx0, pl.dx0, pl.ncopy, rq->clip_limit, rq->tiles,
diff --git a/solex_ser_recon_en_amd/csrc/shg_common.h b/solex_ser_recon_en_amd/csrc/shg_common.h
--- a/solex_ser_recon_en_amd/csrc/shg_common.h
+++ b/solex_ser_recon_en_amd/csrc/shg_common.h
@@ -65,9 +65,10 @@
 int on_frame_pass_lane(hipStream_t st, lane_launch_fn launch, void* arg);
 
 extern thread_local bool t_minmax_slots_zeroed;
-extern thread_local void* t_zero_with_fold;
-extern thread_local size_t t_zero_with_fold_words;
+extern thread_local void* t_zero_with_plan;
+extern thread_local size_t t_zero_with_plan_words;
 extern thread_local void* t_prezeroed;
+extern thread_local bool t_extrema_read_from_slots;
 size_t limb_prepare_zero_words(int64_t h, int64_t w);
 int prelaunch_on_lane(hipStream_t after, lane_launch_fn launch, void* arg, hipEvent_t* done);
 
@@ -119,7 +120,7 @@
                             const double* stats5 = nullptr, double g_bright = 0.0, double g_dark = 0.0, double* mirror5 = nullptr);
 int warp_rows_batch(const uint16_t* const* host_srcs, int64_t k, int64_t h, int64_t w, int64_t src_pitch, const double* host_h3,
                     uint16_t* const* host_dsts, int64_t out_h, int64_t out_w, int64_t dst_pitch, const uint32_t* const* host_minmax2,
-                    shg_stream_t stream);
+                    shg_stream_t stream, bool minmax_slots = false);
 struct FrameSource {
     const uint16_t* const* host_raw;
     int64_t raw_pitch;
diff --git a/solex_ser_recon_en_amd/csrc/stages.hip b/solex_ser_recon_en_amd/csrc/stages.hip
--- a/solex_ser_recon_en_amd/csrc/stages.hip
+++ b/solex_ser_recon_en_amd/csrc/stages.hip
@@ -44,6 +44,8 @@
     size_t n_words;
     uint32_t* zero;
     size_t zero_words;
+    uint32_t* zero2;
+    size_t zero2_words;
 };
 __global__ __launch_bounds__(256) void k_words(const WordsArgs kargs) {
     uint32_t* __restrict__ dst = kargs.dst;
@@ -59,6 +61,8 @@
     uint32_t* __restrict__ zero = kargs.zero;
     for (size_t i = (size_t)blockIdx.x * 256 + threadIdx.x; i < n_words; i += (size_t)gridDim.x * 256) dst[i] = src[i];
     for (size_t i = (size_t)blockIdx.x * 256 + threadIdx.x; i < zero_words; i += (size_t)gridDim.x * 256) zero[i] = 0;
+    uint32_t* __restrict__ zero2 = kargs.zero2;
+    for (size_t i = (size_t)blockIdx.x * 256 + threadIdx.x; i < kargs.zero2_words; i += (size_t)gridDim.x * 256) zero2[i] = 0;
 }
 
 __global__ __launch_bounds__(256) void k_edge_list(const int32_t* __restrict__ comp, int64_t n, int32_t* __restrict__ dst) {
@@ -223,10 +227,16 @@
     const char* end = dense ? reinterpret_cast<const char*>(h_base + ih) : reinterpret_cast<const char*>(h_w2 + 2 * ih);
     if (minmax_slots) {
         const size_t n_words = ((size_t)(end - reinterpret_cast<const char*>(h_ind)) + 3) / 4, zero_words = (size_t)n_shifts * 130;
-        const unsigned blocks = (unsigned)std::min<size_t>((std::max(n_words, zero_words) + 255) / 256, 64);
+        uint32_t* zero2 = static_cast<uint32_t*>(shg::t_zero_with_plan);
+        const size_t zero2_words = zero2 ? shg::t_zero_with_plan_words : 0;
+        shg::t_zero_with_plan = nullptr;
+        shg::t_zero_with_plan_words = 0;
+        const unsigned blocks = (unsigned)std::min<size_t>((std::max(std::max(n_words, zero_words), zero2_words) + 255) / 256, 64);
         STAGE_TRY(shg::launch(k_words_zero, dim3(blocks), dim3(256), 0, st,
-                             WordsArgs{reinterpret_cast<uint32_t*>(ind_l), reinterpret_cast<const uint32_t*>(stg.on_device(h_ind)), n_words, minmax_slots, zero_words}, "k_words_zero"));
+                             WordsArgs{reinterpret_cast<uint32_t*>(ind_l), reinterpret_cast<const uint32_t*>(stg.on_device(h_ind)), n_words, minmax_slots, zero_words,
+                                       zero2, zero2_words}, "k_words_zero"));
         shg::t_minmax_slots_zeroed = true;
+        if (zero2_words) shg::t_prezeroed = zero2;
     } else {
         STAGE_TRY(move_words(ind_l, stg.on_device(h_ind), (size_t)(end - reinterpret_cast<const char*>(h_ind)), st));
     }
@@ -461,7 +471,7 @@
 extern "C" size_t shg_stage_process_workspace_bytes(int64_t k, int64_t h, int64_t w, int64_t crop_w, int tiles) {
     if (k <= 0 || h <= 0 || w <= 0) return 0;
     const size_t pitch = ((size_t)std::max(w, crop_w) + 63) / 64 * 64;
-    return 2 * up((size_t)h * 4) + 2 * up((size_t)k * h * 8) + up((size_t)k * h * 8) + up(4096 * 8) +
+    return 2 * up((size_t)k * h * 8) + up((size_t)k * h * 8) +
            (size_t)k * up((size_t)h * pitch * 2) + (size_t)k * up(shg_contrast_stats_workspace_bytes_for(h, crop_w > 0 ? crop_w : w, tiles)) + up((size_t)k * 5 * 8) + kAlign;
 }
 
@@ -488,9 +498,6 @@
     SHG_REQUIRE(out_pitch >= out_w, SHG_E_ARG, "shg_stage_process_frames: out_pitch < output width");
     hipStream_t st = shg::as_stream(stream);
     Arena dev(workspace, workspace_bytes), pin(host_pinned, host_pinned_bytes);
-    int32_t* xa = dev.take<int32_t>((size_t)h);
-    int32_t* xb = dev.take<int32_t>((size_t)h);
-    double* taps_d = dev.take<double>(4096);
     double* stats = dev.take<double>((size_t)k * h);
     double* interior = dev.take<double>((size_t)k * h);
     double* factors = dev.take<double>((size_t)k * h);
@@ -514,7 +521,7 @@
     double* h_interior = pin.take<double>((size_t)k * h);
     double* h_factors = pin.take<double>((size_t)k * h);
     double* h_out5 = pin.take<double>((size_t)k * 5);
-    SHG_REQUIRE(xa && xb && stats && interior && factors && taps_d && cs_ws && out5 && (!need_tmp || scaled[k - 1]), SHG_E_WORKSPACE,
+    SHG_REQUIRE(stats && interior && factors && cs_ws && out5 && (!need_tmp || scaled[k - 1]), SHG_E_WORKSPACE,
                 "shg_stage_process_frames: workspace too small");
     SHG_REQUIRE(h_xa && h_xb && h_stats && h_interior && h_factors && h_out5 && h_taps, SHG_E_WORKSPACE, "shg_stage_process_frames: pinned staging area too small");
     Staging stg;
@@ -541,9 +548,8 @@
                 for (int64_t i = 0; i < window; ++i) rev[i] = host_taps[window - 1 - i];
                 memcpy(h_taps, rev.data(), (size_t)window * 8);
             }
-            const char* plan_end = gpu_interior ? reinterpret_cast<const char*>(h_taps + window) : reinterpret_cast<const char*>(h_xb + n);
-            STAGE_TRY(move_words(xa, stg.on_device(h_xa), (size_t)(plan_end - reinterpret_cast<const char*>(h_xa)), st));
-            STAGE_TRY(shg::rowpair_stats_batch(host_frames, k, h, w, pitch, y1, y2, xa, xb, nullptr, stats, stg.on_device(h_stats), stream));
+            STAGE_TRY(shg::rowpair_stats_batch(host_frames, k, h, w, pitch, y1, y2, stg.on_device(h_xa), stg.on_device(h_xb), nullptr, stats,
+                                               stg.on_device(h_stats), stream));
             if (gpu_interior) {
                 const int radius = (int)(window / 2);
                 int sym = 1, anti = 1;
@@ -551,7 +557,7 @@
                     if (fabs(rev[radius + i] - rev[radius - i]) > 2.220446049250313e-16) sym = 0;
                     if (fabs(rev[radius + i] + rev[radius - i]) > 2.220446049250313e-16) anti = 0;
                 }
-                STAGE_TRY(shg_correlate1d_rows_f64(stats, k, n, taps_d, radius, sym ? 1 : (anti ? -1 : 0), stg.on_device(h_interior), stream));
+                STAGE_TRY(shg_correlate1d_rows_f64(stats, k, n, stg.on_device(h_taps), radius, sym ? 1 : (anti ? -1 : 0), stg.on_device(h_interior), stream));
                 use_interior = h_interior;
             }
             STAGE_SYNC(st, "shg_stage_process_frames");
diff --git a/solex_ser_recon_en_amd/csrc/transversalium.hip b/solex_ser_recon_en_amd/csrc/transversalium.hip
--- a/solex_ser_recon_en_amd/csrc/transversalium.hip
+++ b/solex_ser_recon_en_amd/csrc/transversalium.hip
@@ -553,11 +553,14 @@
     double* ws = corr_lds + 256 + 2 * radius;
     const int64_t row = blockIdx.y, x0 = (int64_t)blockIdx.x * 256;
     const double* line = src + row * n;
+    const int nw = 2 * radius + 1;
+    const double w_first = (int)threadIdx.x < nw ? weights[threadIdx.x] : 0.0;
     for (int i = threadIdx.x; i < 256 + 2 * radius; i += 256) {
         const int64_t xx = x0 - radius + i;
         xs[i] = (xx >= 0 && xx < n) ? line[xx] : 0.0;
     }
-    for (int i = threadIdx.x; i < 2 * radius + 1; i += 256) ws[i] = weights[i];
+    if ((int)threadIdx.x < nw) ws[threadIdx.x] = w_first;
+    for (int i = threadIdx.x + 256; i < nw; i += 256) ws[i] = weights[i];
     __syncthreads();
     const int64_t x = x0 + threadIdx.x;
     if (x >= n) return;
diff --git a/solex_ser_recon_en_amd/csrc/warp.hip b/solex_ser_recon_en_amd/csrc/warp.hip
--- a/solex_ser_recon_en_amd/csrc/warp.hip
+++ b/solex_ser_recon_en_amd/csrc/warp.hip
@@ -60,7 +60,16 @@
     int64_t out_h, out_w, dst_pitch;
     WarpPtrs mms;
     uint32_t nv_magic, nv_shift;
+    int mm_slots;
 };
+
+__device__ __forceinline__ void warp_extrema(const uint32_t* __restrict__ mm, int slots, uint32_t& lo, uint32_t& hi) {
+    if (!slots) { lo = mm[0]; hi = mm[1]; return; }
+    const uint2 s = reinterpret_cast<const uint2*>(mm)[threadIdx.x & 63];
+    const uint32_t a = shg::wave_fold_u32(s.x, [](uint32_t x, uint32_t y) { return x > y ? x : y; });
+    hi = shg::wave_fold_u32(s.y, [](uint32_t x, uint32_t y) { return x > y ? x : y; });
+    lo = 0xffffu - a;
+}
 
 template <int WARP_ROWS>
 __global__ __launch_bounds__(256) void k_warp_rows(const WarpArgs kargs) {
@@ -75,6 +84,8 @@
     const double h00 = rows.h[blockIdx.z][0], h01 = rows.h[blockIdx.z][1], h02 = rows.h[blockIdx.z][2];
     const int c = (int)(blockIdx.x * 256 + threadIdx.x);
     const int ra = (int)blockIdx.y * WARP_ROWS;
+    uint32_t mm_lo, mm_hi;
+    warp_extrema(mm, kargs.mm_slots, mm_lo, mm_hi);
     if (c >= out_w) return;
     double dc[WARP_ROWS];
     uint32_t v0[WARP_ROWS], v1[WARP_ROWS];
@@ -98,7 +109,7 @@
         v1[rr] = row[in1[rr] ? i1 : 0];
     }
     const uint32_t cval = src[0];
-    const double lo = (double)mm[0], hi = (double)mm[1];
+    const double lo = (double)mm_lo, hi = (double)mm_hi;
 #pragma unroll
     for (int rr = 0; rr < WARP_ROWS; ++rr) {
         const int r = ra + rr;
@@ -125,7 +136,9 @@
     const int lane = threadIdx.x & 63, wave = threadIdx.x >> 6;
     uint32_t (*const my)[64] = win[wave];
     const uint32_t cval = src[0];
-    const int lo_i = (int)mm[0], hi_i = (int)mm[1];
+    uint32_t mm_lo, mm_hi;
+    warp_extrema(mm, kargs.mm_slots, mm_lo, mm_hi);
+    const int lo_i = (int)mm_lo, hi_i = (int)mm_hi;
     const double k00 = h00 * 0x1p+52;
     const uint32_t wu = (uint32_t)w;
     const int w_last = (int)w - 1, last_piece = (int)pitch - 8;
@@ -253,12 +266,14 @@
 
 int shg::warp_rows_batch(const uint16_t* const* host_srcs, int64_t k, int64_t h, int64_t w, int64_t src_pitch, const double* host_h3,
                          uint16_t* const* host_dsts, int64_t out_h, int64_t out_w, int64_t dst_pitch, const uint32_t* const* host_minmax2,
-                         shg_stream_t stream) {
+                         shg_stream_t stream, bool minmax_slots) {
     SHG_REQUIRE(host_srcs && host_h3 && host_dsts && host_minmax2 && k > 0, SHG_E_ARG, "shg_warp_rows_minmax_u16: null pointer");
     SHG_REQUIRE(h > 0 && w > 0 && out_h > 0 && out_w > 0, SHG_E_ARG, "shg_warp_rows_minmax_u16: empty image");
     SHG_REQUIRE(src_pitch >= w && dst_pitch >= out_w, SHG_E_ARG, "shg_warp_rows_minmax_u16: pitch smaller than width");
     SHG_REQUIRE(out_h < 65536 && out_w < (1ll << 30) && w < (1ll << 30) && h < (1ll << 30), SHG_E_UNSUPPORTED, "shg_warp_rows_minmax_u16: image too large");
     for (int64_t i = 0; i < k; ++i) SHG_REQUIRE(host_srcs[i] && host_dsts[i] && host_minmax2[i], SHG_E_ARG, "shg_warp_rows_minmax_u16: null image");
+    for (int64_t i = 0; i < k && minmax_slots; ++i)
+        SHG_REQUIRE((reinterpret_cast<uintptr_t>(host_minmax2[i]) & 7) == 0, SHG_E_ARG, "shg_warp_rows_minmax_u16: extrema slots not 8-byte aligned");
     hipStream_t st = shg::as_stream(stream);
     SHG_PROF("warp", st);
     for (int64_t i0 = 0; i0 < k; i0 += kWarpBatch) {
@@ -271,7 +286,7 @@
         while ((2ull << nv_shift) < nv) ++nv_shift;
         const uint32_t nv_magic = nv >= 2 ? (uint32_t)(((1ull << (32 + nv_shift)) + nv - 1) / nv) : 0u;
         const WarpArgs args{shg::make_batch_n<kWarpBatch>(host_srcs, (int)i0, m), h, w, src_pitch, rows, shg::make_batch_n<kWarpBatch>(host_dsts, (int)i0, m),
-                            out_h, out_w, dst_pitch, shg::make_batch_n<kWarpBatch>(host_minmax2, (int)i0, m), nv_magic, nv_shift};
+                            out_h, out_w, dst_pitch, shg::make_batch_n<kWarpBatch>(host_minmax2, (int)i0, m), nv_magic, nv_shift, minmax_slots ? 1 : 0};
         const bool wide_ok = [] { const char* e = getenv("SHG_WARP_WIDE"); return !e || atoi(e) != 0; }();
         bool wide = wide_ok && src_pitch % 8 == 0 && dst_pitch % 8 == 0 && w >= 8 && src_pitch >= 8 && nv >= 2 && out_h * ((out_w + 7) / 8) < (1ll << 31) &&
                     src_pitch < (1ll << 24) && dst_pitch < (1ll << 24) && h * src_pitch < (1ll << 31) && out_h * dst_pitch < (1ll << 31);
diff --git a/solex_ser_recon_en_amd/stages.py b/solex_ser_recon_en_amd/stages.py
--- a/solex_ser_recon_en_amd/stages.py
+++ b/solex_ser_recon_en_amd/stages.py
@@ -464,7 +464,6 @@
                 out['mask_good'] = self.mask[:max(y2 - y1, 0)].astype(bool)
         if phase >= 2:
             out['disks'] = self.disks[:, :, :n]
-            out['extrema'] = self.mm_store[s * 128:].view(s, 2)
         if phase >= 3:
             out['phi'], out['ratio'] = float(rs.phi), float(rs.ratio)
             out['theta_first'] = float(rs.theta_first)
```
